# hwaranlee/kaldi-cnn

Measured on AMD Instinct MI355X. Metric: frames/sec fwd+bwd, Conv+Maxpool+FC stack, 4096-frame batch @1/2/4/8 GPU, higher is better.
Workload: dtype f32; 1 GPU; c2: Conv(40x11x3, 8x1, 128) -> Maxpool(1x1x4) -> FC(11616->1024), fwd+bwd+update; frames_per_gpu=4096, parallelism=dp1, global_batch=4096, conv_maxpool_fusion=True, conv_output_stored=False

## Files before the change

### include/kcnn.h

```cpp
#ifndef KCNN_KCNN_H_
#define KCNN_KCNN_H_

#include <stddef.h>
#include <stdint.h>

#include "cnsl-hip-kernels.h"

#ifdef __cplusplus
extern "C" {
#endif

const char *kcnn_last_error(void);
const char *kcnn_version(void);
unsigned long long kcnn_device_malloc_calls(void);
int kcnn_conv_fix_counts(unsigned long long *out, int reset);
int kcnn_init(int device);
int kcnn_set_stream(kcnn_stream_t stream);
int kcnn_synchronize(void);
int kcnn_set_literal_path(int literal);
int kcnn_set_profiling(int on);
int kcnn_set_fusion(int mode);
int kcnn_set_gemm_mode(int mode);
int kcnn_gemm_tile_counts(unsigned long long *out, int reset);
int kcnn_gemm_plan(int trans_a, int trans_b, int m, int n, int k, int lda, int ldb, int *out);
int kcnn_gemm_fixup_counts(unsigned long long *out, int reset);
int kcnn_gemm_fixup_sites_reset(void);
int kcnn_set_kernel_family(const char *name, int value);
int kcnn_get_kernel_family(const char *name);
int kcnn_gemm(int trans_a, int trans_b, int m, int n, int k, float alpha,
              const float *a, int lda, const float *b, int ldb, float beta,
              float *c, int ldc);
int kcnn_split_planes(const float *src, int rows, int cols, int ld, uint16_t *dst, int ldp,
                      int64_t ps);
int kcnn_gemm_planes(int trans_a, int trans_b, int m, int n, int k, float alpha,
                     const uint16_t *a, int lda, int64_t aps, const uint16_t *b, int ldb,
                     int64_t bps, float beta, float *c, int ldc);
int kcnn_profile_string(char *buf, size_t len);
int kcnn_reset_profile(void);
void kcnn_set_randn_seed(uint64_t seed);
int kcnn_selftest_fastdiv(void);

int kcnn_mat_conv2d(const float *in, MatrixDim in_dim, const float *kernel,
                    MatrixDim kernel_dim, int in_height, int in_width,
                    int in_channel, int kernel_height, int kernel_width,
                    int group, float *out, MatrixDim out_dim, int concat);
int kcnn_mat_add_mat_rep_vec(float *m, MatrixDim dim, const float *vec,
                             int vec_dim, int rep);
int kcnn_mat_flip_mat(const float *m, MatrixDim dim, int kernel_height,
                      int kernel_width, int in_channel, int group, float *flip,
                      MatrixDim flip_dim);
int kcnn_mat_padding_zero(const float *m, MatrixDim dim, int orig_height,
                          int orig_width, int orig_channel, int kernel_height,
                          int kernel_width, float *padmat, MatrixDim pad_dim);
int kcnn_mat_tp_block(const float *m, MatrixDim dim, int in_channel,
                      int block_size, float *out, MatrixDim out_dim);
int kcnn_mat_tp_inside_block(const float *m, MatrixDim dim, int group,
                             int block_size, float *out, MatrixDim out_dim);
int kcnn_mat_mod_permute_row(const float *m, MatrixDim dim, int in_channel,
                             int block_size, float *out, MatrixDim out_dim);
int kcnn_mat_mod_permute_channel(float *comp, MatrixDim dim, int comp_idx,
                                 int num_component, int in_height, int in_width,
                                 float *container, MatrixDim container_dim,
                                 int from_comp_to_container);
int kcnn_mat_maxpool_prop(const float *in, MatrixDim in_dim, int in_height,
                          int in_width, int pool_height_dim,
                          int pool_width_dim, int pool_channel_dim,
                          int overlap, int overlap2D, float *out,
                          MatrixDim out_dim);
int kcnn_mat_maxpool_backprop(const float *in_value, MatrixDim in_dim,
                              const float *out_value, MatrixDim ov_dim,
                              const float *out_deriv, MatrixDim od_dim,
                              float *in_deriv, MatrixDim id_dim, int in_height,
                              int in_width, int pool_height_dim,
                              int pool_width_dim, int pool_channel_dim,
                              int overlap, int overlap2D);

typedef struct kcnn_component kcnn_component;

kcnn_component *kcnn_component_new_from_string(const char *initializer_line);
kcnn_component *kcnn_component_read(const char *path);
int kcnn_component_write(const kcnn_component *c, const char *path, int binary);
kcnn_component *kcnn_component_copy(const kcnn_component *c);
void kcnn_component_free(kcnn_component *c);
int kcnn_component_type(const kcnn_component *c, char *buf, size_t len);
int kcnn_component_info(const kcnn_component *c, char *buf, size_t len);
int kcnn_component_input_dim(const kcnn_component *c);
int kcnn_component_output_dim(const kcnn_component *c);
int kcnn_component_context(const kcnn_component *c, int *offsets, int max_len);
int kcnn_component_nonlinear_stats(const kcnn_component *c, double *value_sum,
                                   double *deriv_sum, int max_len, int *len,
                                   double *count);
int kcnn_component_backprop_needs_input(const kcnn_component *c);
int kcnn_component_backprop_needs_output(const kcnn_component *c);
int kcnn_component_propagate(const kcnn_component *c, const float *in,
                             MatrixDim in_dim, float *out, MatrixDim out_dim,
                             int num_chunks);
int kcnn_component_backprop(kcnn_component *c, const float *in_value,
                            MatrixDim in_dim, const float *out_value,
                            MatrixDim ov_dim, const float *out_deriv,
                            MatrixDim od_dim, float *in_deriv,
                            MatrixDim id_dim, int num_chunks, int update);
int kcnn_component_param_dim(const kcnn_component *c, int which, int *rows,
                             int *cols);
int kcnn_component_get_param(const kcnn_component *c, int which, float *dst,
                             MatrixDim dst_dim);
int kcnn_component_set_param(kcnn_component *c, int which, const float *src,
                             MatrixDim src_dim);
float kcnn_component_learning_rate(const kcnn_component *c);
// ... 98 lines not shown
```

### kaldi-cnn_amd/kcnn.py

```python
from __future__ import annotations

import ctypes
import os

_HERE = os.path.dirname(os.path.abspath(__file__))
LIB_PATH = os.environ.get("KCNN_LIB") or os.path.join(_HERE, "libkcnn.so")
INCLUDE_DIR = os.path.join(os.path.dirname(_HERE), "include")


class KcnnError(RuntimeError):
    """A KALDI_ASSERT / KALDI_ERR / HIP error raised inside libkcnn.so."""


class MatrixDim(ctypes.Structure):
    _fields_ = [("rows", ctypes.c_int32), ("cols", ctypes.c_int32),
                ("stride", ctypes.c_int32)]

    def __repr__(self):
        return f"MatrixDim({self.rows}, {self.cols}, {self.stride})"


_lib = None


# ... 84 lines not shown

_initialized_device = None


def init(device: int = 0):
    global _initialized_device
    import torch
    if not torch.cuda.is_available():
        raise KcnnError("no GPU: the kcnn product path has no CPU fallback")
    torch.cuda.set_device(device)
    check(lib().kcnn_init(device))
    sync_stream()
    _initialized_device = device


def sync_stream():
    import torch
    check(lib().kcnn_set_stream(ctypes.c_void_p(torch.cuda.current_stream().cuda_stream)))


def _ensure_init():
    if _initialized_device is None:
        import torch
        init(torch.cuda.current_device() if torch.cuda.is_available() else 0)


def set_literal_path(on: bool):
    check(lib().kcnn_set_literal_path(int(bool(on))))


def set_profiling(on: bool):
    check(lib().kcnn_set_profiling(int(bool(on))))


def set_fusion(mode):
    check(lib().kcnn_set_fusion(int(mode)))


def device_malloc_calls() -> int:
    return int(lib().kcnn_device_malloc_calls())


def conv_fix_counts(reset=False):
    if not hasattr(lib(), "kcnn_conv_fix_counts"):
        return None
    out = (ctypes.c_ulonglong * 3)()
    check(lib().kcnn_conv_fix_counts(out, int(bool(reset))))
    return tuple(int(v) for v in out)


def profile_string() -> str:
    buf = ctypes.create_string_buffer(1 << 16)
    check(lib().kcnn_profile_string(buf, len(buf)))
    return buf.value.decode()


def set_gemm_mode(mode: int):
    check(lib().kcnn_set_gemm_mode(int(mode)))


def gemm_tile_counts(reset=False):
    out = (ctypes.c_ulonglong * 2)()
    check(lib().kcnn_gemm_tile_counts(out, int(bool(reset))))
    return tuple(int(v) for v in out)


def gemm_plan(trans_a, trans_b, m, n, k, lda=None, ldb=None):
    if lda is None:
        lda = m if trans_a else k
    if ldb is None:
        ldb = k if trans_b else n
    out = (ctypes.c_int * 3)()
    check(lib().kcnn_gemm_plan(int(bool(trans_a)), int(bool(trans_b)), int(m), int(n), int(k),
                               int(lda), int(ldb), out))
    return tuple(int(v) for v in out)


def gemm_fixup_counts(reset=False):
    out = (ctypes.c_ulonglong * 2)()
    check(lib().kcnn_gemm_fixup_counts(out, int(bool(reset))))
    return tuple(int(v) for v in out)


def gemm_fixup_sites_reset():
    check(lib().kcnn_gemm_fixup_sites_reset())


def set_kernel_family(name: str, value: int):
    check(lib().kcnn_set_kernel_family(name.encode(), int(value)))


def get_kernel_family(name: str) -> int:
    v = lib().kcnn_get_kernel_family(name.encode())
    if v < 0:
        raise KcnnError(f"unknown kernel family {name!r}")
    return v


def gemm(a, b, c, trans_a=False, trans_b=False, alpha=1.0, beta=0.0):
    m, n = c.shape
    am, k = (a.shape[1], a.shape[0]) if trans_a else (a.shape[0], a.shape[1])
    bk, bn = (b.shape[1], b.shape[0]) if trans_b else (b.shape[0], b.shape[1])
    if am != m or bk != k or bn != n:
        raise KcnnError(f"gemm: op(a) {am}x{k}, op(b) {bk}x{bn} do not make c {m}x{n}")
    for t in (a, b, c):
        dim(t)
    check(lib().kcnn_gemm(int(bool(trans_a)), int(bool(trans_b)), m, n, k,
                          ctypes.c_float(alpha), ctypes.c_void_p(a.data_ptr()), a.stride(0),
                          ctypes.c_void_p(b.data_ptr()), b.stride(0), ctypes.c_float(beta),
                          ctypes.c_void_p(c.data_ptr()), c.stride(0)))


def split_planes(x):
    import torch
    rows, cols = x.shape
    ldp = (cols + 7) // 8 * 8
    out = torch.zeros((3, rows, ldp), dtype=torch.int16, device=x.device)
    check(lib().kcnn_split_planes(ctypes.c_void_p(x.data_ptr()), rows, cols, x.stride(0),
                                  ctypes.c_void_p(out.data_ptr()), ldp,
                                  ctypes.c_int64(rows * ldp)))
    return out


def gemm_planes(ap, bp, c, k, trans_a=False, trans_b=False, alpha=1.0, beta=0.0):
    m, n = c.shape
    check(lib().kcnn_gemm_planes(int(bool(trans_a)), int(bool(trans_b)), m, n, k,
                                 ctypes.c_float(alpha), ctypes.c_void_p(ap.data_ptr()),
                                 ap.stride(1), ctypes.c_int64(ap.stride(0)),
                                 ctypes.c_void_p(bp.data_ptr()), bp.stride(1),
                                 ctypes.c_int64(bp.stride(0)), ctypes.c_float(beta),
                                 ctypes.c_void_p(c.data_ptr()), c.stride(0)))


def reset_profile():
    check(lib().kcnn_reset_profile())


def set_randn_seed(seed: int):
    lib().kcnn_set_randn_seed(ctypes.c_uint64(seed))


def synchronize():
    check(lib().kcnn_synchronize())


def dim(t) -> MatrixDim:
    assert t.dim() == 2, "matrices are 2-D"
    assert t.dtype.is_floating_point and t.element_size() == 4, t.dtype
    assert t.is_cuda, "device tensors only"
    assert t.shape[1] <= 1 or t.stride(1) == 1, "rows must be contiguous"
    stride = t.stride(0) if t.shape[0] > 1 else max(t.shape[1], 1)
    return MatrixDim(t.shape[0], t.shape[1], stride)


def ptr(t):
    return ctypes.c_void_p(t.data_ptr()) if t is not None else None


def empty(rows, cols, device=None):
    import torch
    return torch.empty((rows, cols), dtype=torch.float32,
                       device=device or "cuda")


def zeros(rows, cols, device=None):
    import torch
# ... 668 lines not shown
```

### kaldi-cnn_amd/src/capi/kcnn-capi.cc

```cpp
#include "kcnn.h"

#include <stdlib.h>
#include <string.h>

#include <algorithm>
#include <fstream>
#include <sstream>
#include <string>
#include <utility>
#include <vector>

#include "../cnslmat/hip-util.h"
#include "../kaldi-lite/cu-device.h"
#include "../kaldi-lite/cu-kernels-lite.h"
#include "../kaldi-lite/cu-matrix.h"
#include "../kaldi-lite/kaldi-io.h"
#include "../nnet0/nnet-component-nnet0.h"
#include "../nnet2/nnet-component.h"
#include "../nnet2/nnet-kernels.h"
#include "nnet-stack.h"
#include "online-computer.h"
#include "xent-labels.h"

using namespace kaldi;
// ... 1 lines not shown

struct kcnn_nnet {
  kcnn::NnetStack stack;
  template <typename... Args>
  explicit kcnn_nnet(Args &&...args) : stack(std::forward<Args>(args)...) {}
};

struct kcnn_corpus {
  const float *feats = nullptr;
  MatrixDim dim = {0, 0, 0};
  kcnn::CorpusIndex index;
};

struct kcnn_online {
  kcnn::OnlineComputer computer;
  template <typename... Args>
  explicit kcnn_online(Args &&...args) : computer(std::forward<Args>(args)...) {}
};

namespace {
thread_local std::string g_err;

int fail(const char *what) {
  g_err = what;
  return -1;
}

template <typename F>
int guard(F f) {
  try {
    f();
    return 0;
  } catch (const std::exception &e) {
    return fail(e.what());
  } catch (...) {
    return fail("unknown C++ exception");
  }
}

CuSubMatrix<BaseFloat> view(const float *p, MatrixDim d) {
  return CuSubMatrix<BaseFloat>(const_cast<float *>(p), d.rows, d.cols, d.stride);
}

void borrow(CuMatrix<BaseFloat> *m, const float *p, MatrixDim d) {
  m->Borrow(const_cast<float *>(p), d.rows, d.cols, d.stride);
}

ChunkInfo chunk_info(int cols, int rows, int num_chunks) {
  if (num_chunks <= 0) num_chunks = rows;
  KALDI_ASSERT(rows > 0 && rows % num_chunks == 0);
  return ChunkInfo(cols, num_chunks, 0, rows / num_chunks - 1);
}

void component_chunks(const Component *c, MatrixDim in_dim, MatrixDim out_dim,
                      int num_chunks, ChunkInfo *ii, ChunkInfo *oi) {
  const std::vector<int32> ctx = c->Context();
  if (num_chunks <= 0) num_chunks = out_dim.rows;
  KALDI_ASSERT(out_dim.rows > 0 && out_dim.rows % num_chunks == 0 &&
               in_dim.rows % num_chunks == 0);
  const int ocs = out_dim.rows / num_chunks;
  KALDI_ASSERT(in_dim.rows / num_chunks == ocs + ctx.back() - ctx.front());
  *oi = ChunkInfo(out_dim.cols, num_chunks, 0, ocs - 1);
  if (ctx.front() == 0 && ctx.back() == 0) {
    *ii = ChunkInfo(in_dim.cols, num_chunks, 0, ocs - 1);
  } else {
    *oi = ChunkInfo(out_dim.cols, num_chunks, -ctx.front(), ocs - 1 - ctx.front());
    *ii = ChunkInfo(in_dim.cols, num_chunks, 0, ocs - 1 + ctx.back() - ctx.front());
  }
}

void copy_out(std::string s, char *buf, size_t len) {
  if (!buf || !len) return;
  strncpy(buf, s.c_str(), len - 1);
  buf[len - 1] = '\0';
}

UpdatableComponent *updatable(const kcnn_component *c) {
  KALDI_ASSERT(c && c->c);
  UpdatableComponent *u = dynamic_cast<UpdatableComponent *>(c->c);
  if (!u) KALDI_ERR << c->c->Type() << " has no parameters";
  return u;
}

void param_ref(const kcnn_component *c, int which, float **data, MatrixDim *dim) {
  using cnsl::nnet0::ConvolutionComponent;
  using cnsl::nnet0::FullyConnectedComponent;
  CuMatrixBase<BaseFloat> *m = nullptr;
  CuVectorBase<BaseFloat> *v = nullptr;
  if (auto *cc = dynamic_cast<ConvolutionComponent *>(c->c)) {
    if (which == 0) m = &cc->LinearParamsMutable();
    else if (which == 1) v = &cc->BiasParamsMutable();
    else if (which == 2) m = &cc->PrevGradMutable();
  } else if (auto *fc = dynamic_cast<FullyConnectedComponent *>(c->c)) {
    if (which == 0) m = &fc->LinearParamsMutable();
    else if (which == 1) v = &fc->BiasParamsMutable();
    else if (which == 2) m = &fc->PrevGradMutable();
  } else if (auto *af = dynamic_cast<AffineComponent *>(c->c)) {
    if (which == 0) m = &af->LinearParamsMutable();
    else if (which == 1) v = &af->BiasParamsMutable();
  }
  if (m) {
    *data = m->Data();
    *dim = m->Dim();
  } else if (v) {
    *data = v->Data();
    dim->rows = 1; dim->cols = v->Dim(); dim->stride = v->Dim();
  } else {
    KALDI_ERR << c->c->Type() << " has no parameter #" << which;
  }
}

void copy2d(float *dst, MatrixDim dd, const float *src, MatrixDim sd) {
  KALDI_ASSERT(dd.rows == sd.rows && dd.cols == sd.cols);
  if (dd.rows == 0 || dd.cols == 0) return;
  CU_SAFE_CALL(hipMemcpy2DAsync(dst, sizeof(float) * dd.stride, src,
                                sizeof(float) * sd.stride,
                                sizeof(float) * dd.cols, dd.rows,
                                hipMemcpyDeviceToDevice,
                                CuDevice::Instantiate().Stream()));
}

kcnn::NnetStack &stack(const kcnn_nnet *n) { return const_cast<kcnn_nnet *>(n)->stack; }

void matrix_out(const CuMatrix<BaseFloat> &m, const float **data, MatrixDim *dim) {
  *data = m.Data();
  *dim = m.Dim();
}
}

extern "C" {

const char *kcnn_last_error(void) { return g_err.c_str(); }
const char *kcnn_version(void) { return "kcnn-mi355x 0.1 (gfx950)"; }
unsigned long long kcnn_device_malloc_calls(void) {
  return (unsigned long long)CuDevice::Instantiate().MallocCalls();
}

int kcnn_init(int device) {
  return guard([&] { CuDevice::Instantiate().SelectGpuId("yes", device); });
}
int kcnn_set_stream(kcnn_stream_t stream) {
  return guard([&] {
    CuDevice::Instantiate().SetStream(reinterpret_cast<hipStream_t>(stream));
  });
}
int kcnn_synchronize(void) {
  return guard([&] { CuDevice::Instantiate().Synchronize(); });
}
int kcnn_set_literal_path(int literal) {
  cnsl::nnet0::SetLiteralPath(literal != 0);
  return 0;
}
int kcnn_set_fusion(int on) {
  if (on < 0 || on > 2) return fail("kcnn_set_fusion: mode is 0, 1 or 2");
  kcnn::set_fusion_mode(on);
  return 0;
}
int kcnn_set_gemm_mode(int mode) {
  if (mode < 0 || mode > 4) return fail("kcnn_set_gemm_mode: mode is 0 to 4");
  CuDevice::Instantiate().SetGemmMode(mode);
  return 0;
}
int kcnn_gemm_tile_counts(unsigned long long *out, int reset) {
  if (!out) return fail("kcnn_gemm_tile_counts: out is NULL");
  kl_gemm_f16x3_tile_counts(out, reset);
  return 0;
}
int kcnn_gemm_plan(int trans_a, int trans_b, int m, int n, int k, int lda, int ldb, int *out) {
  if (!out) return fail("kcnn_gemm_plan: out is NULL");
  if (m <= 0 || n <= 0 || k <= 0) return fail("kcnn_gemm_plan: dimensions must be positive");
  kl_gemm_f16x3_plan(trans_a, trans_b, m, n, k, lda, ldb, out);
  return 0;
}
int kcnn_gemm_fixup_counts(unsigned long long *out, int reset) {
  if (!out) return fail("kcnn_gemm_fixup_counts: out is NULL");
  kl_gemm_f16x3_fixup_counts(out, reset);
  return 0;
}
int kcnn_gemm_fixup_sites_reset(void) {
  kl_gemm_f16x3_fixup_sites_reset();
  return 0;
}
int kcnn_set_kernel_family(const char *name, int value) {
  const int f = kcnn::family_by_name(name);
  if (f < 0) return fail("kcnn_set_kernel_family: unknown family");
  if (kcnn::set_family(static_cast<kcnn::Family>(f), value) != 0)
    return fail("kcnn_set_kernel_family: value out of range");
  return 0;
}
int kcnn_get_kernel_family(const char *name) {
  const int f = kcnn::family_by_name(name);
  return f < 0 ? -1 : kcnn::family(static_cast<kcnn::Family>(f));
}
int kcnn_gemm(int trans_a, int trans_b, int m, int n, int k, float alpha,
              const float *a, int lda, const float *b, int ldb, float beta,
              float *c, int ldc) {
  return guard([&] {
    if (m < 0 || n < 0 || k < 0) KALDI_ERR << "kcnn_gemm: negative dimension";
    const int ar = trans_a ? k : m, ac = trans_a ? m : k;
    const int br = trans_b ? n : k, bc = trans_b ? k : n;
    if (lda < ac || ldb < bc || ldc < n) KALDI_ERR << "kcnn_gemm: leading dimension too small";
    CuSubMatrix<BaseFloat> A(const_cast<float *>(a), ar, ac, lda);
    CuSubMatrix<BaseFloat> B(const_cast<float *>(b), br, bc, ldb);
    CuSubMatrix<BaseFloat> C(c, m, n, ldc);
    C.AddMatMat(alpha, A, trans_a ? kTrans : kNoTrans, B, trans_b ? kTrans : kNoTrans, beta);
  });
}
int kcnn_split_planes(const float *src, int rows, int cols, int ld, uint16_t *dst, int ldp,
                      int64_t ps) {
  return guard([&] {
    CuDevice &d = CuDevice::Instantiate();
    const int rc = kl_split_planes(src, rows, cols, ld, dst, ldp, ps,
                                   reinterpret_cast<kcnn_stream_t>(d.Stream()));
    if (rc) KALDI_ERR << "kcnn_split_planes: " << hipGetErrorString((hipError_t)rc);
  });
}
int kcnn_gemm_planes(int trans_a, int trans_b, int m, int n, int k, float alpha,
                     const uint16_t *a, int lda, int64_t aps, const uint16_t *b, int ldb,
                     int64_t bps, float beta, float *c, int ldc) {
  return guard([&] {
    CuDevice &d = CuDevice::Instantiate();
    const size_t wsb = kl_gemm_planes_workspace_bytes(m, n, k);
    CuScratch ws_s(wsb);
    void *ws = ws_s.p;
    const int rc = kl_gemm_planes(trans_a, trans_b, m, n, k, alpha, a, lda, aps, b, ldb, bps,
                                  beta, c, ldc, ws, wsb,
                                  reinterpret_cast<kcnn_stream_t>(d.Stream()));
    if (rc) KALDI_ERR << "kcnn_gemm_planes: " << hipGetErrorString((hipError_t)rc);
  });
}
int kcnn_set_profiling(int on) {
  CuDevice::Instantiate().SetProfiling(on != 0);
  return 0;
}
int kcnn_profile_string(char *buf, size_t len) {
  return guard([&] { copy_out(CuDevice::Instantiate().ProfileString(), buf, len); });
}
int kcnn_reset_profile(void) {
  return guard([&] {
    CuDevice &d = CuDevice::Instantiate();
    (void)d.ProfileString();
    d.ResetProfile();
  });
}
void kcnn_set_randn_seed(uint64_t seed) { SetRandnSeed(seed); }

int kcnn_selftest_fastdiv(void) {
  const uint32_t divs[] = {1, 2, 3, 5, 7, 8, 11, 24, 33, 40, 128, 363, 440,
                           1320, 11616, 46464, 65535, 1000003, 0x7fffffffu};
  uint64_t state = 12345;
  for (uint32_t d : divs) {
    kcnn::FastDiv f(d);
    for (int t = 0; t < 20000; t++) {
      state = state * 6364136223846793005ull + 1442695040888963407ull;
      uint32_t n = (uint32_t)(state >> 33);
      if (t < 64) n = (uint32_t)t;
      if (t >= 64 && t < 128) n = 0x7fffffffu - (uint32_t)(t - 64);
      uint32_t q, r;
      f.divmod(n, q, r);
// ... 160 lines not shown
  guard([&] {
    const std::vector<int32> ctx = c->c->Context();
    n = (int)ctx.size();
    for (int k = 0; k < n && k < max_len; k++) offsets[k] = ctx[k];
  });
  return n;
}
int kcnn_component_nonlinear_stats(const kcnn_component *c, double *value_sum,
                                   double *deriv_sum, int max_len, int *len,
                                   double *count) {
  return guard([&] {
    auto *nl = dynamic_cast<const kaldi::nnet2::NonlinearComponent *>(c->c);
    if (!nl) KALDI_ERR << c->c->Type() << " is not a NonlinearComponent";
    Vector<double> v, d;
    nl->GetValueSum(&v);
    nl->GetDerivSum(&d);
    *len = v.Dim();
    for (int k = 0; k < v.Dim() && k < max_len; k++) {
      value_sum[k] = v(k);
      deriv_sum[k] = d(k);
    }
    *count = nl->Count();
  });
}
int kcnn_component_backprop_needs_input(const kcnn_component *c) {
  return c->c->BackpropNeedsInput();
}
int kcnn_component_backprop_needs_output(const kcnn_component *c) {
  return c->c->BackpropNeedsOutput();
}

int kcnn_component_propagate(const kcnn_component *c, const float *in,
                             MatrixDim in_dim, float *out, MatrixDim out_dim,
                             int num_chunks) {
  return guard([&] {
    auto x = view(in, in_dim), y = view(out, out_dim);
    ChunkInfo ii, oi;
    component_chunks(c->c, in_dim, out_dim, num_chunks, &ii, &oi);
    c->c->Propagate(ii, oi, x, &y);
  });
}

int kcnn_component_backprop(kcnn_component *c, const float *in_value,
                            MatrixDim in_dim, const float *out_value,
                            MatrixDim ov_dim, const float *out_deriv,
                            MatrixDim od_dim, float *in_deriv,
                            MatrixDim id_dim, int num_chunks, int update) {
  return guard([&] {
    auto x = view(in_value, in_dim), y = view(out_value, ov_dim),
         dy = view(out_deriv, od_dim);
    ChunkInfo ii, oi;
    component_chunks(c->c, in_dim, od_dim, num_chunks, &ii, &oi);
    CuMatrix<BaseFloat> dx;
    if (in_deriv) borrow(&dx, in_deriv, id_dim);
    Component *to_update = update ? c->c : nullptr;
    c->c->Backprop(ii, oi, x, y, dy, to_update, in_deriv ? &dx : nullptr);
  });
}

int kcnn_component_param_dim(const kcnn_component *c, int which, int *rows,
                             int *cols) {
  return guard([&] {
    float *p;
    MatrixDim d;
    param_ref(c, which, &p, &d);
    *rows = d.rows;
    *cols = d.cols;
  });
}
int kcnn_component_get_param(const kcnn_component *c, int which, float *dst,
                             MatrixDim dst_dim) {
  return guard([&] {
    float *p;
    MatrixDim d;
    param_ref(c, which, &p, &d);
    copy2d(dst, dst_dim, p, d);
  });
}
int kcnn_component_set_param(kcnn_component *c, int which, const float *src,
                             MatrixDim src_dim) {
  return guard([&] {
    float *p;
    MatrixDim d;
    param_ref(c, which, &p, &d);
    copy2d(p, d, src, src_dim);
  });
}
float kcnn_component_learning_rate(const kcnn_component *c) {
  float lr = -1.0f;
  guard([&] { lr = updatable(c)->LearningRate(); });
  return lr;
}
int kcnn_component_set_learning_rate(kcnn_component *c, float lr) {
  return guard([&] { updatable(c)->SetLearningRate(lr); });
}
int kcnn_component_dot_product(const kcnn_component *a, const kcnn_component *b,
                               float *out) {
  return guard([&] { *out = updatable(a)->DotProduct(*updatable(b)); });
}
int kcnn_component_set_zero(kcnn_component *c, int treat_as_gradient) {
  return guard([&] { updatable(c)->SetZero(treat_as_gradient != 0); });
}
int kcnn_component_scale(kcnn_component *c, float scale) {
  return guard([&] { updatable(c)->Scale(scale); });
}
int kcnn_component_add(kcnn_component *c, float alpha, const kcnn_component *other) {
  return guard([&] { updatable(c)->Add(alpha, *updatable(other)); });
}
int kcnn_component_perturb_params(kcnn_component *c, float stddev) {
  return guard([&] { updatable(c)->PerturbParams(stddev); });
}
int kcnn_component_num_gradient_params(const kcnn_component *c) {
  auto *u = dynamic_cast<UpdatableComponent *>(c->c);
  return u ? u->NumGradientParams() : 0;
}
int kcnn_component_compute_gradient(const kcnn_component *c,
                                    const float *in_value, MatrixDim in_dim,
                                    const float *out_deriv, MatrixDim od_dim,
                                    float *grad) {
  return guard([&] {
    updatable(c)->ComputeGradient(view(in_value, in_dim), view(out_deriv, od_dim),
                                  grad);
  });
}
int kcnn_component_apply_gradient(kcnn_component *c, const float *grad,
                                  int num_sample) {
  return guard([&] { updatable(c)->ApplyGradient(grad, num_sample); });
}
int kcnn_component_backprop_gradient(const kcnn_component *c,
                                     const float *in_value, MatrixDim in_dim,
                                     const float *out_deriv, MatrixDim od_dim,
                                     float *in_deriv, MatrixDim id_dim,
                                     float *grad) {
  return guard([&] {
    const UpdatableComponent *u = updatable(c);
    ChunkInfo ii = chunk_info(in_dim.cols, in_dim.rows, 0);
    ChunkInfo oi = chunk_info(od_dim.cols, od_dim.rows, 0);
    auto x = view(in_value, in_dim);
    CuMatrix<BaseFloat> dx;
    if (in_deriv) borrow(&dx, in_deriv, id_dim);
    u->BackpropGradient(ii, oi, x, x, view(out_deriv, od_dim),
                        in_deriv ? &dx : nullptr, grad);
  });
}
int kcnn_component_conv_flip_branch(const kcnn_component *c) {
  auto *cc = dynamic_cast<cnsl::nnet0::ConvolutionComponent *>(c->c);
  if (!cc) return fail("not a ConvolutionComponent");
  return cc->FlipKernelBranch() ? 1 : 0;
}

namespace {
DropoutComponent *dropout(const kcnn_component *c) {
  KALDI_ASSERT(c && c->c);
  DropoutComponent *d = dynamic_cast<DropoutComponent *>(c->c);
  if (!d) KALDI_ERR << c->c->Type() << " is not a DropoutComponent";
  return d;
}
}

int kcnn_component_set_dropout_scale(kcnn_component *c, float scale) {
  return guard([&] { dropout(c)->SetDropoutScale(scale); });
}
int kcnn_component_dropout_seed(const kcnn_component *c, uint64_t *seed) {
  return guard([&] { *seed = dropout(c)->Seed(); });
}
int kcnn_component_set_dropout_seed(kcnn_component *c, uint64_t seed) {
  return guard([&] { dropout(c)->SetSeed(seed); });
// ... 256 lines not shown
```

### kaldi-cnn_amd/src/capi/nnet-stack.cc

```cpp
#include "nnet-stack.h"

#include <stdlib.h>

#include <cmath>
#include <set>
#include <sstream>
#include <string>

#include "../kaldi-lite/kaldi-io.h"
#include "../nnet2/nnet-kernels.h"
#include "xent-labels.h"

using namespace kaldi;
using namespace kaldi::nnet2;

namespace kcnn {

namespace {
int g_fusion = [] {
  const char *e = getenv("KCNN_FUSE");
  return e && *e ? atoi(e) : 1;
}();

void size_output(CuMatrix<BaseFloat> *m, int rows, int cols) {
// ... 363 lines not shown
}

void NnetStack::MaterialisePoolDeriv(int i) {
  Comp &c = comps_[i];
  KALDI_ASSERT(c.pool != NULL && c.mask_valid && i + 1 < NumComponents());
  c.pool->BackpropFromMask(static_cast<unsigned char *>(c.mask.p), c.pool->OutputDim(),
                           out_deriv_of(i, nullptr, MatrixDim()), &c.deriv);
  c.deriv_deferred = false;
}

const CuMatrix<BaseFloat> &NnetStack::InputDeriv(int i) {
  KALDI_ASSERT(i >= 0 && i < NumComponents());
  if (i == 0 && frames_fused_)
    KALDI_ERR << "input derivative of component 0: after kcnn_nnet_propagate_frames a first "
              << "SpliceComponent reads the corpus itself and its Backprop is not run (it has "
              << "no parameters, and examples share corpus rows)";
  if (comps_[i].deriv_deferred) MaterialisePoolDeriv(i);
  return comps_[i].deriv;
}

void NnetStack::BackpropComponent(int i, const float *out_deriv, MatrixDim od_dim,
                                  BackpropMode mode, float *grad, bool skip_first_dx) {
  const int nc = NumComponents();
  KALDI_ASSERT(i >= 0 && i < nc);
  RequireTrainingForward("kcnn_nnet_backprop_component");
  RequireLastNotFused(i, "kcnn_nnet_backprop_component");
  if (i == 0 && frames_fused_) return;
  Comp &c = comps_[i];
  auto hint = input_stats(i);
  if (out(i).stale == kRecomputable) out(i).stale = kGone;
  const CuMatrix<BaseFloat> &x = in(i).value, &y = out(i).value;
  const bool pool_above_deferred = i + 1 < nc && comps_[i + 1].deriv_deferred;
  CuMatrix<BaseFloat> *dx = &c.deriv;
  if (i == 0 && skip_first_dx && c.updatable) dx = nullptr;
  if (mode == kGradientOnly) {
    KALDI_ASSERT(c.updatable != NULL && grad != NULL && !pool_above_deferred && !c.mask_valid);
    c.updatable->BackpropGradient(in_info(i), out_info(i), x, y,
                                  out_deriv_of(i, out_deriv, od_dim), nullptr, grad);
    return;
  }
  if (pool_above_deferred) {
    const Comp &p = comps_[i + 1];
    if (c.conv && p.pool &&
        c.conv->BackpropPooled(x, *p.pool, static_cast<unsigned char *>(p.mask.p),
                               p.pool->OutputDim(), out_deriv_of(i + 1, out_deriv, od_dim),
                               to_update(c, mode), dx, mode == kGradient ? grad : nullptr))
      return;
    MaterialisePoolDeriv(i + 1);
  }
  CuSubMatrix<BaseFloat> od = out_deriv_of(i, out_deriv, od_dim);
  ChunkInfo ii = in_info(i), oi = out_info(i);
  if (mode == kGradient && c.updatable) {
    c.updatable->BackpropGradient(ii, oi, x, y, od, dx, grad);
    return;
  }
  if (c.mask_valid) {
    KALDI_ASSERT(c.pool != NULL);
    if (g_fusion == 1 && i < nc - 1 && c.pool->FoldsIntoConvBackprop()) {
      c.deriv_deferred = true;
      return;
    }
    c.pool->BackpropFromMask(static_cast<unsigned char *>(c.mask.p), c.pool->OutputDim(), od,
                             dx);
    return;
  }
  c.c->Backprop(ii, oi, x, y, od, to_update(c, mode), dx);
}

void NnetStack::BackpropSplit(int i, const float *out_deriv, MatrixDim od_dim, float *grad,
                              bool skip_first_dx, void (*between)(void *), void *ctx) {
  const int nc = NumComponents();
  KALDI_ASSERT(i >= 0 && i < nc && grad != NULL);
  RequireTrainingForward("kcnn_nnet_backprop_split");
  RequireLastNotFused(i, "kcnn_nnet_backprop_split");
  Comp &c = comps_[i];
  if (c.affine == NULL) KALDI_ERR << "kcnn_nnet_backprop_split: component " << i << " is not affine";
  KALDI_ASSERT(!(i + 1 < nc && comps_[i + 1].deriv_deferred) && !c.mask_valid);
  auto hint = input_stats(i);
  if (out(i).stale == kRecomputable) out(i).stale = kGone;
  const CuMatrix<BaseFloat> &x = in(i).value, &y = out(i).value;
  CuSubMatrix<BaseFloat> od = out_deriv_of(i, out_deriv, od_dim);
  CuMatrix<BaseFloat> *dx = (i == 0 && skip_first_dx) ? nullptr : &c.deriv;
  ChunkInfo ii = in_info(i), oi = out_info(i);
  CuGemmBackpropStats stats(od, c.affine->LinearParams(), true, &x);
  c.affine->BackpropGradient(ii, oi, x, y, od, nullptr, grad);
  if (between) between(ctx);
  if (dx) c.c->Backprop(ii, oi, x, y, od, to_update(c, kDataOnly), dx);
}

void NnetStack::Backprop(const float *out_deriv, MatrixDim od_dim) {
  for (int i = NumComponents() - 1; i >= 0; i--)
    BackpropComponent(i, out_deriv, od_dim, kUpdate, nullptr, false);
}

double *NnetStack::objf_totals() {
  kaldi::CuBuffer &t = labels_.totals;
  if (!t.p)
    CU_SAFE_CALL(hipMemsetAsync(t.reserve(2 * sizeof(double)), 0, 2 * sizeof(double),
                                CuDevice::Instantiate().Stream()));
  return static_cast<double *>(t.p);
}

const char *NnetStack::LabelStaging::Stage(const int32_t *rows, const int32_t *cols,
                                           const float *weights, int num, int num_rows,
                                           hipStream_t st) {
  const size_t bytes = label_layout(num, num_rows).bytes;
  stage_labels(rows, cols, weights, num, num_rows, Begin(bytes));
  return Commit(bytes, st);
}

char *NnetStack::LabelStaging::Begin(size_t bytes) {
  if (copied == nullptr)
    CU_SAFE_CALL(hipEventCreateWithFlags(&copied, hipEventDisableTiming));
  else
    CU_SAFE_CALL(hipEventSynchronize(copied));
  if (host_bytes < bytes) {
    if (host) CU_SAFE_CALL(hipHostFree(host));
    host = nullptr;
    host_bytes = 0;
    CU_SAFE_CALL(hipHostMalloc(&host, bytes, hipHostMallocDefault));
    host_bytes = bytes;
  }
  return static_cast<char *>(host);
}

const char *NnetStack::LabelStaging::Commit(size_t bytes, hipStream_t st) {
  dev.reserve(bytes);
  CU_SAFE_CALL(hipMemcpyAsync(dev.p, host, bytes, hipMemcpyHostToDevice, st));
  CU_SAFE_CALL(hipEventRecord(copied, st));
  return static_cast<const char *>(dev.p);
}

int NnetStack::XentDeriv(const int32_t *rows, const int32_t *cols, const float *weights,
                         int num, const float **out_deriv, MatrixDim *od_dim,
                         const char *who) {
  const int nc = NumComponents();
  RequireTrainingForward(who);
  const Comp &last = comps_[nc - 1];
  const CuMatrix<BaseFloat> &y = out(nc - 1).value;
  const int N = y.NumRows(), dim = last.c->OutputDim();
  if (N == 0 || y.NumCols() != dim) KALDI_ERR << who << ": no Propagate ran";
  if (num > 0 && weights == nullptr) KALDI_ERR << who << ": bad label arrays";
  const std::string bad = check_labels(rows, cols, num, N, dim, true);
  if (!bad.empty()) KALDI_ERR << who << ": " << bad;
  const DeviceLabels lab = StageLabels(rows, cols, weights, num, N);
  const int32_t *d_start = lab.row_start, *d_row = lab.row, *d_col = lab.col;
  const float *d_w = lab.weight;
  double *tot = objf_totals();
  if (last.softmax != nullptr && !cnsl::nnet0::LiteralPath()) {
    last.softmax->BackpropXent(y, d_start, d_col, d_w, tot, last.softmax,
                               &comps_[nc - 1].deriv);
    xent_fused_ = true;
    *out_deriv = nullptr;
    *od_dim = MatrixDim{0, 0, 0};
    return nc - 2;
  }
  xent_deriv_.Resize(N, dim, kSetZero);
  if (num > 0)
    comp_objf_and_deriv(d_row, d_col, d_w, num, y.Data(), y.Dim(), xent_deriv_.Data(),
                        xent_deriv_.Dim(), tot);
  *out_deriv = xent_deriv_.Data();
  *od_dim = xent_deriv_.Dim();
  return nc - 1;
}

void NnetStack::BackpropXent(const int32_t *rows, const int32_t *cols, const float *weights,
// ... 274 lines not shown
```

### kaldi-cnn_amd/src/kaldi-lite/cu-f16-stats.hip

```cpp
#include <hip/hip_runtime.h>
#include <stdint.h>

#include <algorithm>

#include "cnslmat/f16-split.h"
#include "cnslmat/hip-util.h"
#include "cnslmat/pool-stats-dev.h"
#include "cnslmat/pool-stats.h"
#include "kaldi-lite/cu-kernels-lite.h"
#include "kaldi-lite/f16-stats.h"

using namespace kcnn::f16x3;

namespace {

using kcnn::COLMAX_ROWS;
using kcnn::PoolCountSmem;
using kcnn::pool_colmax_block;
using kcnn::pool_count_block;

__device__ __forceinline__ const float *X_row(const StatOp &o, int r) {
  return o.X + (int64_t)r * o.ld;
}

// ... 27 lines not shown
  const int lane = threadIdx.x & 63, wave = threadIdx.x >> 6;
  const bool wide = o.rpb == 1;
  const int r = wide ? blk : blk * 4 + wave;
  if (r >= o.rows) return;
  const float *x = X_row(o, r);
  const int step = wide ? 1024 : 256;
  const int c0 = (wide ? threadIdx.x : lane) * 4;
  const bool held = o.vec && o.cols <= RV * step;
  float4 q[RV];
  uint32_t m = 0, n = 0xffffffffu;
  if (held) {
#pragma unroll
    for (int j = 0; j < RV; ++j) {
      const int c = c0 + j * step;
      if (c + 4 <= o.cols) {
        q[j] = *reinterpret_cast<const float4 *>(x + c);
      } else {
        q[j].x = c < o.cols ? x[c] : 0.0f;
        q[j].y = c + 1 < o.cols ? x[c + 1] : 0.0f;
        q[j].z = c + 2 < o.cols ? x[c + 2] : 0.0f;
        q[j].w = 0.0f;
      }
    }
#pragma unroll
    for (int j = 0; j < RV; ++j) mm4(m, n, q[j]);
  } else {
    int c = c0;
    if (o.vec) {
      for (; c + 3 * step + 4 <= o.cols; c += 4 * step) {
        float4 v[4];
#pragma unroll
        for (int j = 0; j < 4; ++j) v[j] = *reinterpret_cast<const float4 *>(x + c + j * step);
#pragma unroll
        for (int j = 0; j < 4; ++j) mm4(m, n, v[j]);
      }
      for (; c + 4 <= o.cols; c += step) mm4(m, n, *reinterpret_cast<const float4 *>(x + c));
    }
    for (; c < o.cols; c += step)
#pragma unroll
      for (int i = 0; i < 4; ++i)
        if (c + i < o.cols) mm1(m, n, x[c + i]);
  }
#pragma unroll
  for (int d = 32; d >= 1; d >>= 1) {
    m = max(m, (uint32_t)__shfl_xor((int)m, d));
    n = min(n, (uint32_t)__shfl_xor((int)n, d));
  }
  if (wide) {
    if (lane == 0) {
      red[wave] = m;
      red[4 + wave] = n;
    }
    __syncthreads();
    m = max(max(red[0], red[1]), max(red[2], red[3]));
    n = min(min(red[4], red[5]), min(red[6], red[7]));
  }
  uint32_t cnt = 0;
  if (kcnn::f16x3::spread(m, n + 1u)) {
    const float bound = kcnn::f16x3::small_bound(m);
    if (held) {
      auto small = [&](float v) { return (fabsf(v) < bound && v != 0.0f) ? 1u : 0u; };
#pragma unroll
      for (int j = 0; j < RV; ++j)
        cnt += small(q[j].x) + small(q[j].y) + small(q[j].z) + small(q[j].w);
    } else {
      cnt = count_small_row(o, x, bound, c0, step);
    }
#pragma unroll
    for (int d = 32; d >= 1; d >>= 1) cnt += (uint32_t)__shfl_xor((int)cnt, d);
    if (wide) {
      __syncthreads();
      if (lane == 0) red[8 + wave] = cnt;
      __syncthreads();
      cnt = red[8] + red[9] + red[10] + red[11];
    }
  }
  if (wide ? threadIdx.x == 0 : lane == 0) {
    o.out[r] = m;
    o.out[o.rows + r] = n + 1u;
    o.out[2 * (size_t)o.rows + r] = cnt;
  }
}

__device__ __forceinline__ void stats_cols(const StatOp &o, int blk) {
  const int cbi = blk % o.cb, rci = blk / o.cb;
  const int c0 = cbi * 1024 + threadIdx.x * 4;
  const int r0 = rci * o.rb, rend = min(o.rows, r0 + o.rb);
  if (c0 >= o.cols) return;
  const bool v4 = o.vec && c0 + 4 <= o.cols;
  uint32_t cm[4] = {0u, 0u, 0u, 0u};
  uint32_t cn[4] = {0xffffffffu, 0xffffffffu, 0xffffffffu, 0xffffffffu};
  auto load = [&](int r) {
    const float *x = X_row(o, r) + c0;
    if (v4) return *reinterpret_cast<const float4 *>(x);
    float4 q;
    q.x = x[0];
    q.y = c0 + 1 < o.cols ? x[1] : 0.0f;
    q.z = c0 + 2 < o.cols ? x[2] : 0.0f;
    q.w = c0 + 3 < o.cols ? x[3] : 0.0f;
    return q;
  };
  auto take = [&](float4 q) {
    mm1(cm[0], cn[0], q.x);
    mm1(cm[1], cn[1], q.y);
    mm1(cm[2], cn[2], q.z);
    mm1(cm[3], cn[3], q.w);
  };
  int r = r0;
  for (; r + 8 <= rend; r += 8) {
    float4 q[8];
#pragma unroll
    for (int j = 0; j < 8; ++j) q[j] = load(r + j);
#pragma unroll
    for (int j = 0; j < 8; ++j) take(q[j]);
  }
  for (; r < rend; ++r) take(load(r));
  uint32_t *dst = o.part + (size_t)rci * o.cols + c0;
  uint32_t *dsn = dst + (size_t)o.rbk * o.cols;
#pragma unroll
  for (int i = 0; i < 4; ++i)
    if (c0 + i < o.cols) {
      dst[i] = cm[i];
      dsn[i] = cn[i];
    }
}

struct StatOps {
  StatOp o[3];
  PoolColDeferred pc;
  int pcx, pcy, pcn;
};
template <typename Count>
__device__ __forceinline__ int pick_op(const StatOps &s, int blk, Count count, int &local) {
  const int n0 = count(s.o[0]), n1 = count(s.o[1]);
  if (blk < n0) { local = blk; return 0; }
  if (blk < n0 + n1) { local = blk - n0; return 1; }
  local = blk - n0 - n1;
  return 2;
}
__host__ __device__ inline int ncount_blocks(const StatOp &o);
__host__ __device__ inline int nfinal_blocks(const StatOp &o) {
  return o.mode == 1 && o.blocks ? o.fblocks : 0;
}

__global__ __launch_bounds__(256) void stats_kernel(StatOps s) {
  __shared__ uint32_t red[12];
  if (s.o[0].clear && blockIdx.x == 0 && threadIdx.x < 2) s.o[0].clear[threadIdx.x] = 0u;
  const int nb3 = s.o[0].blocks + s.o[1].blocks + s.o[2].blocks;
  if ((int)blockIdx.x >= nb3) {
    const int k = blockIdx.x - nb3;
    pool_colmax_block(s.pc.pcol, s.pc.nblk, s.pc.npool, s.pc.colblk, k % s.pcx, k / s.pcx);
    return;
  }
  int blk;
  const int w = pick_op(s, blockIdx.x, [](const StatOp &o) { return o.blocks; }, blk);
  const StatOp &o = s.o[w];
  if (o.mode == 0) stats_rows(o, blk, red);
  else stats_cols(o, blk);
}

__global__ __launch_bounds__(256) void stats_finalize_kernel(StatOps s) {
  __shared__ uint32_t red[2][4][64];
  __shared__ PoolCountSmem psm;
  const int nf3 = nfinal_blocks(s.o[0]) + nfinal_blocks(s.o[1]) + nfinal_blocks(s.o[2]);
  if ((int)blockIdx.x >= nf3) {
    pool_count_block(s.pc.P, s.pc.ps, s.pc.R, s.pc.npool, s.pc.vec, s.pc.rowblk, s.pc.colblk,
                     blockIdx.x - nf3, s.pcn, psm);
    return;
  }
  int blk;
  const StatOp &o = s.o[pick_op(s, blockIdx.x, [](const StatOp &q) { return nfinal_blocks(q); }, blk)];
  const int lane = threadIdx.x & 63, grp = threadIdx.x >> 6;
  const int c = blk * 64 + lane;
  uint32_t m = 0, n = 0xffffffffu;
  if (c < o.cols) {
    const uint32_t *pm = o.part + c, *pn = o.part + (size_t)o.rbk * o.cols + c;
    int q = grp;
    for (; q + 28 < o.rbk; q += 32) {
      uint32_t a[8], b[8];
#pragma unroll
      for (int j = 0; j < 8; ++j) {
        a[j] = pm[(size_t)(q + 4 * j) * o.cols];
        b[j] = pn[(size_t)(q + 4 * j) * o.cols];
      }
#pragma unroll
      for (int j = 0; j < 8; ++j) {
        m = max(m, a[j]);
        n = min(n, b[j]);
      }
    }
    for (; q < o.rbk; q += 4) {
      m = max(m, pm[(size_t)q * o.cols]);
      n = min(n, pn[(size_t)q * o.cols]);
    }
  }
  red[0][grp][lane] = m;
  red[1][grp][lane] = n;
  __syncthreads();
  m = max(max(red[0][0][lane], red[0][1][lane]), max(red[0][2][lane], red[0][3][lane]));
  n = min(min(red[1][0][lane], red[1][1][lane]), min(red[1][2][lane], red[1][3][lane]));
  if (grp == 0 && c < o.cols) {
    o.out[c] = m;
    o.out[o.cols + c] = n + 1u;
    o.out[2 * (size_t)o.cols + c] = 0;
  }
}

constexpr int CNT_ROWS = 64;
__host__ __device__ inline int ncount_blocks(const StatOp &o) {
  return o.mode == 1 && o.blocks ? ((o.cols + 63) / 64) * ((o.rows + CNT_ROWS - 1) / CNT_ROWS) : 0;
}
__global__ __launch_bounds__(256) void stats_count_kernel(StatOps s) {
  int blk;
  const StatOp &o = s.o[pick_op(s, blockIdx.x, [](const StatOp &q) { return ncount_blocks(q); }, blk)];
  const int ncb = (o.cols + 63) / 64;
  const int cb = blk % ncb, rc = blk / ncb;
  const int lane = threadIdx.x & 63, wave = threadIdx.x >> 6;
  const int c = cb * 64 + lane;
  bool spr = false;
  float bound = 0.0f;
  if (c < o.cols) {
    const uint32_t mx = o.out[c];
    spr = kcnn::f16x3::spread(mx, o.out[o.cols + c]);
    if (spr) bound = kcnn::f16x3::small_bound(mx);
  }
  if (__ballot(spr) == 0) return;
  const int r0 = rc * CNT_ROWS, r1 = min(o.rows, r0 + CNT_ROWS);
  uint32_t cnt = 0;
  if (spr) {
    float v[CNT_ROWS / 4];
#pragma unroll
    for (int i = 0; i < CNT_ROWS / 4; ++i) {
      const int r = r0 + wave + 4 * i;
      v[i] = r < r1 ? fabsf(X_row(o, r)[c]) : 0.0f;
    }
#pragma unroll
    for (int i = 0; i < CNT_ROWS / 4; ++i) cnt += (v[i] < bound && v[i] != 0.0f) ? 1u : 0u;
  }
  if (cnt) atomicAdd(o.out + 2 * (size_t)o.cols + c, cnt);
}

int stats_launch3(const StatOps &ops, hipStream_t st) {
  for (const StatOp &o : ops.o)
    if (o.blocks == 0 && o.out) {
      const size_t n = o.mode == 0 ? (size_t)std::max(o.rows, 0) : (size_t)std::max(o.cols, 0);
      if (n && hipMemsetAsync(o.out, 0, 3 * n * 4, st) != hipSuccess) return (int)hipGetLastError();
    }
  int nb = 0, nf = 0, nc = 0;
  for (const StatOp &o : ops.o) {
    nb += o.blocks;
    nf += nfinal_blocks(o);
    nc += ncount_blocks(o);
  }
  nb += ops.pcx * ops.pcy;
  nf += ops.pcn;
  if (nb == 0) return 0;
  hipLaunchKernelGGL(stats_kernel, dim3(nb), dim3(256), 0, st, ops);
  int rc = kcnn::launch_status();
  if (rc || nf == 0) return rc;
  hipLaunchKernelGGL(stats_finalize_kernel, dim3(nf), dim3(256), 0, st, ops);
  rc = kcnn::launch_status();
  if (rc || nc == 0) return rc;
  hipLaunchKernelGGL(stats_count_kernel, dim3(nc), dim3(256), 0, st, ops);
  return kcnn::launch_status();
}

}

namespace kcnn::f16x3 {

StatOp stat_op(const float *X, int rows, int cols, int ld, int mode, uint32_t *out,
               uint32_t *part) {
  StatOp o{};
  o.X = X; o.out = out; o.part = part;
  o.rows = rows; o.cols = cols; o.ld = ld; o.mode = mode;
  o.vec = ld % 4 == 0 && (uintptr_t)X % 16 == 0;
  if (rows <= 0 || cols <= 0) return o;
  if (mode == 0) {
    o.rpb = cols >= 2048 ? 1 : 4;
    o.blocks = (rows + o.rpb - 1) / o.rpb;
  } else {
    o.cb = (cols + 1023) / 1024;
    o.rbk = std::max(1, std::min(256, std::min((rows + 15) / 16, (1024 + o.cb - 1) / o.cb)));
    o.rb = (rows + o.rbk - 1) / o.rbk;
    o.rbk = (rows + o.rb - 1) / o.rb;
    o.blocks = o.cb * o.rbk;
    o.fblocks = (cols + 63) / 64;
  }
  return o;
}
size_t stat_part_words(int rows, int cols, int mode) {
  if (mode == 0) return 0;
  const StatOp o = stat_op(nullptr, rows, cols, cols, 1, nullptr, nullptr);
  return 2 * (size_t)o.rbk * cols;
}
int stats_launch(const StatOp &a, const StatOp &b, hipStream_t st) {
  StatOps ops{};
  ops.o[0] = a;
  ops.o[1] = b;
  ops.o[2] = StatOp{};
  return stats_launch3(ops, st);
}

}

extern "C" int kl_absmax_rows(const float *X, int rows, int cols, int ld, uint32_t *rmax,
                              kcnn_stream_t stream) {
  if (rows < 0 || cols < 0 || ld < cols || !rmax) return (int)hipErrorInvalidValue;
  return stats_launch(stat_op(X, rows, cols, ld, 0, rmax, nullptr), StatOp{},
                      kcnn::as_stream(stream));
}
extern "C" size_t kl_absmax_cols_words(int rows, int cols) {
  if (rows <= 0 || cols <= 0) return 0;
  return stat_part_words(rows, cols, 1);
}
extern "C" int kl_absmax_cols(const float *X, int rows, int cols, int ld, uint32_t *cmax,
                              uint32_t *part, kcnn_stream_t stream) {
  if (rows < 0 || cols < 0 || ld < cols || !cmax) return (int)hipErrorInvalidValue;
  if (rows > 0 && cols > 0 && !part) return (int)hipErrorInvalidValue;
  return stats_launch(stat_op(X, rows, cols, ld, 1, cmax, part), StatOp{},
                      kcnn::as_stream(stream));
}

extern "C" int kl_absmax_rows_cols(const float *R, int rows, int cols, int ld, uint32_t *rmax,
                                   const float *Q, int qrows, int qcols, int ldq, uint32_t *cmax,
                                   uint32_t *part, uint32_t *clear, kcnn_stream_t stream) {
  if (rows < 0 || cols < 0 || ld < cols || !rmax || qrows < 0 || qcols < 0 || ldq < qcols ||
      !cmax)
    return (int)hipErrorInvalidValue;
  if (qrows > 0 && qcols > 0 && !part) return (int)hipErrorInvalidValue;
  StatOp q = stat_op(Q, qrows, qcols, ldq, 1, cmax, part);
  q.clear = clear;
  const StatOp r = stat_op(R, rows, cols, ld, 0, rmax, nullptr);
  if (clear && q.blocks + r.blocks == 0) {
    const hipError_t e = hipMemsetAsync(clear, 0, 8, kcnn::as_stream(stream));
    if (e != hipSuccess) return (int)e;
  }
  return stats_launch(q, r, kcnn::as_stream(stream));
}

extern "C" int kl_gemm_stats3(const float *X0, int rows0, int cols0, int ld0, int mode0,
                              uint32_t *out0, uint32_t *part0, const float *X1, int rows1,
                              int cols1, int ld1, int mode1, uint32_t *out1, uint32_t *part1,
                              const float *X2, int rows2, int cols2, int ld2, int mode2,
                              uint32_t *out2, uint32_t *part2, void *pool_cols,
                              kcnn_stream_t stream) {
  StatOps ops{};
  if (pool_cols) {
    ops.pc = *static_cast<const PoolColDeferred *>(pool_cols);
    const int ncq = ops.pc.npool % 4 == 0 ? ops.pc.npool / 4 : ops.pc.npool;
    ops.pcx = (ncq + 255) / 256;
    ops.pcy = (ops.pc.nblk + COLMAX_ROWS - 1) / COLMAX_ROWS;
    ops.pcn = std::min(ops.pc.R, 256);
  }
  const float *X[3] = {X0, X1, X2};
  const int rows[3] = {rows0, rows1, rows2}, cols[3] = {cols0, cols1, cols2};
  const int ld[3] = {ld0, ld1, ld2}, mode[3] = {mode0, mode1, mode2};
  uint32_t *out[3] = {out0, out1, out2}, *part[3] = {part0, part1, part2};
  for (int i = 0; i < 3; ++i) {
    ops.o[i] = StatOp{};
    if (!X[i]) continue;
    if (rows[i] < 0 || cols[i] < 0 || ld[i] < cols[i] || !out[i] || (mode[i] != 0 && mode[i] != 1) ||
        (mode[i] == 1 && rows[i] > 0 && cols[i] > 0 && !part[i]))
      return (int)hipErrorInvalidValue;
    ops.o[i] = stat_op(X[i], rows[i], cols[i], ld[i], mode[i], out[i], mode[i] ? part[i] : nullptr);
  }
  return stats_launch3(ops, kcnn::as_stream(stream));
}
```

### kaldi-cnn_amd/src/kaldi-lite/cu-kernels-lite.h

```cpp
#ifndef KCNN_KALDI_LITE_CU_KERNELS_LITE_H_
#define KCNN_KALDI_LITE_CU_KERNELS_LITE_H_

#include <stddef.h>
#include <stdint.h>

#include "cnsl-hip-kernels.h"

#ifdef __cplusplus
extern "C" {
#endif
int kl_set(float *d, MatrixDim dim, float v, kcnn_stream_t st);
int kl_scale(float *d, MatrixDim dim, float a, kcnn_stream_t st);
int kl_add(float *d, MatrixDim dim, float a, kcnn_stream_t st);
int kl_add_mat(float alpha, const float *A, MatrixDim ad, int transA,
               float beta, float *D, MatrixDim dd, kcnn_stream_t st);
int kl_copy_rows_from_vec(const float *v, float *D, MatrixDim dd,
                          kcnn_stream_t st);
int kl_sum_partials(const float *parts, int S, int m, int n, float beta,
                    float *C, MatrixDim cd, kcnn_stream_t st);
size_t kl_col_sum_workspace_bytes(MatrixDim md);
int kl_col_sum(const float *M, MatrixDim md, float alpha, float beta, float *v,
               void *ws, kcnn_stream_t st);
size_t kl_gemm_x6_workspace_bytes(int M, int N, int K);
int kl_gemm_x6(int transA, int transB, int M, int N, int K, float alpha,
               const float *A, int lda, const float *B, int ldb, float beta,
               float *C, int ldc, void *ws, size_t ws_bytes, kcnn_stream_t st);
int kl_absmax_rows(const float *X, int rows, int cols, int ld, uint32_t *rmax,
                   kcnn_stream_t st);
size_t kl_absmax_cols_words(int rows, int cols);
int kl_absmax_cols(const float *X, int rows, int cols, int ld, uint32_t *cmax, uint32_t *part,
                   kcnn_stream_t st);
int kl_absmax_rows_cols(const float *R, int rows, int cols, int ld, uint32_t *rmax,
                        const float *Q, int qrows, int qcols, int ldq, uint32_t *cmax,
                        uint32_t *part, uint32_t *clear, kcnn_stream_t stream);
int kl_gemm_stats3(const float *X0, int rows0, int cols0, int ld0, int mode0, uint32_t *out0,
                   uint32_t *part0, const float *X1, int rows1, int cols1, int ld1, int mode1,
                   uint32_t *out1, uint32_t *part1, const float *X2, int rows2, int cols2,
                   int ld2, int mode2, uint32_t *out2, uint32_t *part2, void *pool_cols,
                   kcnn_stream_t stream);
size_t kl_gemm_f16x3_workspace_bytes(int M, int N, int K);
void kl_gemm_f16x3_tile_counts(unsigned long long *out, int reset);
size_t kl_gemm_f16x3_plan(int transA, int transB, int M, int N, int K, int lda, int ldb,
                          int *out);
void kl_gemm_f16x3_fixup_counts(unsigned long long *out, int reset);
void kl_gemm_f16x3_fixup_sites_reset(void);
size_t kl_gemm_f16x3_full_workspace_bytes(int M, int N, int K);
int kl_gemm_f16x3(int transA, int transB, int M, int N, int K, float alpha,
                  const float *A, int lda, const float *B, int ldb, float beta, float *C,
                  int ldc, void *ws, size_t ws_bytes, kcnn_stream_t st);
int kl_gemm_f16x3_bias(int transA, int transB, int M, int N, int K, float alpha,
                       const float *A, int lda, const float *B, int ldb, float beta, float *C,
                       int ldc, const uint32_t *amax_given, const uint32_t *bmax_given,
                       const float *bias, void *ws, size_t ws_bytes, kcnn_stream_t stream);
int kl_gemm_f16x3_momentum(int transA, int transB, int M, int N, int K, const float *A,
                           int lda, const float *B, int ldb, const uint32_t *amax_given,
                           const uint32_t *bmax_given, float *W, int ldw, float *prev, int ldp,
                           float momentum, float a_wd, float a_g, void *ws, size_t ws_bytes,
                           kcnn_stream_t stream);
int kl_split_planes(const float *src, int rows, int cols, int ld, uint16_t *dst, int ldp,
                    int64_t ps, kcnn_stream_t st);
size_t kl_gemm_planes_workspace_bytes(int M, int N, int K);
int kl_gemm_planes(int transA, int transB, int M, int N, int K, float alpha,
                   const uint16_t *A, int lda, int64_t aps, const uint16_t *B, int ldb,
                   int64_t bps, float beta, float *C, int ldc, void *ws, size_t ws_bytes,
                   kcnn_stream_t st);
int kl_dot(const float *A, MatrixDim ad, const float *B, MatrixDim bd,
           int transB, double *out_dev, kcnn_stream_t st);
#ifdef __cplusplus
}
#endif
#endif
```

### kaldi-cnn_amd/src/kaldi-lite/cu-matrix.cc

```cpp
#include "cu-matrix.h"

#include <math.h>
#include <stdint.h>
#include <stdlib.h>
#include <string.h>

#include <limits>
#include <mutex>
#include <sstream>

#include "cu-device.h"
#include "cu-kernels-lite.h"
#include "../cnslmat/pool-stats.h"
#include "kaldi-io.h"

namespace kaldi {

namespace {
inline kcnn_stream_t S() {
  return reinterpret_cast<kcnn_stream_t>(CuDevice::Instantiate().Stream());
}
inline MatrixIndexT PaddedStride(MatrixIndexT cols) {
  return (cols + 15) / 16 * 16;
}
::MatrixDim VecDim(MatrixIndexT n) {
  ::MatrixDim d;
  d.rows = 1; d.cols = n; d.stride = n;
  return d;
}

std::mutex g_rng_mu;
uint64_t g_rng_state = 20261015ull;
uint64_t splitmix64() {
  uint64_t z = (g_rng_state += 0x9E3779B97F4A7C15ull);
  z = (z ^ (z >> 30)) * 0xBF58476D1CE4E5B9ull;
  z = (z ^ (z >> 27)) * 0x94D049BB133111EBull;
  return z ^ (z >> 31);
}
}

void SetRandnSeed(uint64_t seed) {
  std::lock_guard<std::mutex> lk(g_rng_mu);
  g_rng_state = seed;
}

uint64_t RandU64() {
  std::lock_guard<std::mutex> lk(g_rng_mu);
  return splitmix64();
}

void RandnFill(float *dst, size_t n) {
  std::lock_guard<std::mutex> lk(g_rng_mu);
  for (size_t i = 0; i < n; i += 2) {
    const double u1 = ((splitmix64() >> 11) + 1.0) * (1.0 / 9007199254740993.0);
    const double u2 = (splitmix64() >> 11) * (1.0 / 9007199254740992.0);
    const double r = sqrt(-2.0 * log(u1));
    dst[i] = (float)(r * cos(2.0 * M_PI * u2));
    if (i + 1 < n) dst[i + 1] = (float)(r * sin(2.0 * M_PI * u2));
  }
}

template <typename Real>
void MatrixBase<Real>::Write(std::ostream &os, bool binary) const {
  if (binary) {
    WriteToken(os, binary, sizeof(Real) == 4 ? "FM" : "DM");
    WriteBasicType(os, binary, (int32)rows_);
    WriteBasicType(os, binary, (int32)cols_);
    os.write(reinterpret_cast<const char *>(data_.data()),
             sizeof(Real) * data_.size());
  } else {
    if (cols_ == 0) {
      os << " [ ]\n";
    } else {
      os << " [";
      os.precision(std::numeric_limits<Real>::max_digits10);
      for (MatrixIndexT i = 0; i < rows_; i++) {
        os << "\n  ";
        for (MatrixIndexT j = 0; j < cols_; j++) os << (*this)(i, j) << " ";
      }
      os << "]\n";
    }
  }
  if (os.fail()) KALDI_ERR << "failed to write matrix";
}

template <typename Real>
void MatrixBase<Real>::Read(std::istream &is, bool binary) {
  if (binary) {
    std::string tok;
// ... 114 lines not shown

template <typename Real>
void CuMatrixBase<Real>::CopyFromMat(const CuMatrixBase<Real> &src,
                                     MatrixTransposeType trans) {
  if (trans == kNoTrans) {
    KALDI_ASSERT(src.NumRows() == num_rows_ && src.NumCols() == num_cols_);
    if (num_rows_ == 0 || num_cols_ == 0) return;
    CU_SAFE_CALL(hipMemcpy2DAsync(data_, sizeof(Real) * stride_, src.Data(),
                                  sizeof(Real) * src.Stride(),
                                  sizeof(Real) * num_cols_, num_rows_,
                                  hipMemcpyDeviceToDevice,
                                  CuDevice::Instantiate().Stream()));
  } else {
    KALDI_ASSERT(src.NumCols() == num_rows_ && src.NumRows() == num_cols_);
    CNSL_SAFE_CALL(kl_add_mat(1.0f, src.Data(), src.Dim(), 1, 0.0f, data_, Dim(), S()));
  }
}

template <typename Real>
void CuMatrixBase<Real>::CopyFromMat(const MatrixBase<Real> &src) {
  KALDI_ASSERT(src.NumRows() == num_rows_ && src.NumCols() == num_cols_);
  if (num_rows_ == 0 || num_cols_ == 0) return;
  CU_SAFE_CALL(hipMemcpy2DAsync(data_, sizeof(Real) * stride_, src.Data(),
                                sizeof(Real) * src.Stride(),
                                sizeof(Real) * num_cols_, num_rows_,
                                hipMemcpyHostToDevice,
                                CuDevice::Instantiate().Stream()));
  CuDevice::Instantiate().Synchronize();
}

template <typename Real>
void CuMatrixBase<Real>::CopyToMat(MatrixBase<Real> *dst) const {
  if (dst->NumRows() != num_rows_ || dst->NumCols() != num_cols_)
    dst->Resize(num_rows_, num_cols_);
  if (num_rows_ == 0 || num_cols_ == 0) return;
  CU_SAFE_CALL(hipMemcpy2DAsync(dst->Data(), sizeof(Real) * dst->Stride(),
                                data_, sizeof(Real) * stride_,
                                sizeof(Real) * num_cols_, num_rows_,
                                hipMemcpyDeviceToHost,
                                CuDevice::Instantiate().Stream()));
  CuDevice::Instantiate().Synchronize();
}

template <typename Real>
void CuMatrixBase<Real>::AddMat(Real alpha, const CuMatrixBase<Real> &A,
                                MatrixTransposeType trans) {
  if (trans == kNoTrans)
    KALDI_ASSERT(A.NumRows() == num_rows_ && A.NumCols() == num_cols_);
  else
    KALDI_ASSERT(A.NumCols() == num_rows_ && A.NumRows() == num_cols_);
  CNSL_SAFE_CALL(kl_add_mat(alpha, A.Data(), A.Dim(), trans == kTrans, 1.0f,
                            data_, Dim(), S()));
}

static thread_local const CuGemmStatsHint *g_stats_hints = nullptr;

CuGemmStatsHint::CuGemmStatsHint(const float *data, MatrixIndexT rows, MatrixIndexT cols,
                                 MatrixIndexT stride, const uint32_t *rmax,
                                 const uint32_t *cmax)
    : rowmax(rmax), colmax(cmax), data_(data), rows_(rows), cols_(cols), stride_(stride),
      prev_(g_stats_hints) {
  g_stats_hints = this;
}
CuGemmStatsHint::~CuGemmStatsHint() { g_stats_hints = prev_; }
const CuGemmStatsHint *CuGemmStatsHint::Find(const float *data, MatrixIndexT rows,
                                             MatrixIndexT cols, MatrixIndexT stride) {
  for (const CuGemmStatsHint *h = g_stats_hints; h; h = h->prev_)
    if (h->data_ == data && h->rows_ == rows && h->cols_ == cols && h->stride_ == stride)
      return h;
  return nullptr;
}

static const uint32_t *hint_cols(const CuGemmStatsHint *h, kcnn_stream_t st) {
  if (h->pending) CNSL_SAFE_CALL(kcnn_pool_cols_complete(h->pending, st));
  return h->colmax;
}

CuGemmBackpropStats::CuGemmBackpropStats(const CuMatrixBase<float> &dy,
                                         const CuMatrixBase<float> &W, bool cols,
                                         const CuMatrixBase<float> *in) {
  CuDevice &dev = CuDevice::Instantiate();
  const int N = dy.NumRows(), O = dy.NumCols(), I = W.NumCols();
  if (dev.GemmMode() < 2 || N == 0 || O == 0 || I == 0 || W.NumRows() != O) return;
  {
    const CuGemmStatsHint *hd = CuGemmStatsHint::Find(dy.Data(), N, O, dy.Stride());
    const CuGemmStatsHint *hw = CuGemmStatsHint::Find(W.Data(), O, I, W.Stride());
    if (hd && hd->rowmax && (!cols || hd->colmax) && hw && hw->colmax && !hw->pending) return;
  }
  const size_t pd = cols ? kl_absmax_cols_words(N, O) : 0, pw = kl_absmax_cols_words(O, I);
  const size_t words = 3 * ((size_t)N + O + I) + pd + pw;
  ws_ = dev.Malloc(words * 4);
  uint32_t *rows_d = static_cast<uint32_t *>(ws_), *cols_d = rows_d + 3 * (size_t)N,
           *cols_w = cols_d + 3 * (size_t)O, *part_d = cols_w + 3 * (size_t)I,
           *part_w = part_d + pd;
  PoolColDeferred *pc = nullptr;
  if (cols && in) {
    const CuGemmStatsHint *h =
        CuGemmStatsHint::Find(in->Data(), in->NumRows(), in->NumCols(), in->Stride());
    if (h && h->pending && h->pending->pending) pc = h->pending;
  }
  CNSL_SAFE_CALL(kl_gemm_stats3(dy.Data(), N, O, dy.Stride(), 0, rows_d, nullptr,
                                cols ? dy.Data() : nullptr, N, O, dy.Stride(), 1, cols_d, part_d,
                                W.Data(), O, I, W.Stride(), 1, cols_w, part_w, pc,
                                reinterpret_cast<kcnn_stream_t>(dev.Stream())));
  if (pc) pc->pending = 0;
  hint_d_ = new CuGemmStatsHint(dy.Data(), N, O, dy.Stride(), rows_d, cols ? cols_d : nullptr);
  hint_w_ = new CuGemmStatsHint(W.Data(), O, I, W.Stride(), nullptr, cols_w);
}
CuGemmBackpropStats::~CuGemmBackpropStats() {
  delete hint_w_;
  delete hint_d_;
  if (ws_) CuDevice::Instantiate().Free(ws_);
}

template <typename Real>
bool CuMatrixBase<Real>::GemmF16x3(Real alpha, const CuMatrixBase<Real> &A,
                                   const CuMatrixBase<Real> &Ap, MatrixTransposeType transA,
                                   const CuMatrixBase<Real> &B, const CuMatrixBase<Real> &Bp,
                                   MatrixTransposeType transB, Real beta, const Real *bias) {
  const MatrixIndexT m = num_rows_, n = num_cols_;
  const MatrixIndexT k = transA == kNoTrans ? A.NumCols() : A.NumRows();
  CuDevice &dev0 = CuDevice::Instantiate();
  const CuGemmStatsHint *ha = CuGemmStatsHint::Find(A.Data(), A.NumRows(), A.NumCols(),
                                                    A.Stride());
  const CuGemmStatsHint *hb = CuGemmStatsHint::Find(B.Data(), B.NumRows(), B.NumCols(),
                                                    B.Stride());
  const uint32_t *ag = ha ? (transA == kNoTrans ? ha->rowmax : hint_cols(ha, S())) : nullptr;
  const uint32_t *bg = hb ? (transB == kNoTrans ? hint_cols(hb, S()) : hb->rowmax) : nullptr;
  const size_t wsf = kl_gemm_f16x3_full_workspace_bytes(m, n, k);
  void *wf = dev0.Malloc(wsf);
  const int rc = kl_gemm_f16x3_bias(transA == kTrans, transB == kTrans, m, n, k, alpha,
                                    Ap.Data(), Ap.Stride(), Bp.Data(), Bp.Stride(), beta, data_,
                                    stride_, ag, bg, bias, wf, wsf, S());
  dev0.Free(wf);
  if (rc == (int)hipErrorNotSupported) return false;
  CNSL_SAFE_CALL(rc);
  return true;
}

template <typename Real>
bool CuMatrixBase<Real>::AddMatMatMomentum(const CuMatrixBase<Real> &A,
                                           MatrixTransposeType transA,
                                           const CuMatrixBase<Real> &B,
                                           MatrixTransposeType transB, CuMatrixBase<Real> *prev,
                                           Real momentum, Real a_wd, Real a_g) {
  const MatrixIndexT m = num_rows_, n = num_cols_;
  const MatrixIndexT k = transA == kNoTrans ? A.NumCols() : A.NumRows();
  CuDevice &dev0 = CuDevice::Instantiate();
  auto aligned = [](const CuMatrixBase<Real> &X) {
    return X.Stride() % 4 == 0 && reinterpret_cast<uintptr_t>(X.Data()) % 16 == 0;
  };
  if (dev0.GemmMode() < 2 || m == 0 || n == 0 || k == 0 || !aligned(A) || !aligned(B) ||
      !aligned(*this) || !aligned(*prev))
    return false;
  KALDI_ASSERT((transA == kNoTrans ? A.NumRows() : A.NumCols()) == m &&
               (transB == kNoTrans ? B.NumCols() : B.NumRows()) == n &&
               (transB == kNoTrans ? B.NumRows() : B.NumCols()) == k &&
               prev->NumRows() == m && prev->NumCols() == n);
  CuProfileScope prof("AddMatMat");
  const CuGemmStatsHint *ha = CuGemmStatsHint::Find(A.Data(), A.NumRows(), A.NumCols(),
                                                    A.Stride());
  const CuGemmStatsHint *hb = CuGemmStatsHint::Find(B.Data(), B.NumRows(), B.NumCols(),
                                                    B.Stride());
  const uint32_t *ag = ha ? (transA == kNoTrans ? ha->rowmax : hint_cols(ha, S())) : nullptr;
  const uint32_t *bg = hb ? (transB == kNoTrans ? hint_cols(hb, S()) : hb->rowmax) : nullptr;
  const size_t wsf = kl_gemm_f16x3_full_workspace_bytes(m, n, k);
  void *wf = dev0.Malloc(wsf);
  const int rc = kl_gemm_f16x3_momentum(transA == kTrans, transB == kTrans, m, n, k, A.Data(),
                                        A.Stride(), B.Data(), B.Stride(), ag, bg, data_, stride_,
                                        prev->Data(), prev->Stride(), momentum, a_wd, a_g, wf,
                                        wsf, S());
  dev0.Free(wf);
  if (rc == (int)hipErrorNotSupported) return false;
  CNSL_SAFE_CALL(rc);
  return true;
}

template <typename Real>
void CuMatrixBase<Real>::AddMatMatBias(Real alpha, const CuMatrixBase<Real> &A,
                                       MatrixTransposeType transA, const CuMatrixBase<Real> &B,
                                       MatrixTransposeType transB,
                                       const CuVectorBase<Real> &bias) {
  const MatrixIndexT k = transA == kNoTrans ? A.NumCols() : A.NumRows();
  KALDI_ASSERT(bias.Dim() == num_cols_);
  CuDevice &dev0 = CuDevice::Instantiate();
  auto aligned = [](const CuMatrixBase<Real> &X) {
    return X.Stride() % 4 == 0 && reinterpret_cast<uintptr_t>(X.Data()) % 16 == 0;
  };
  if (dev0.GemmMode() >= 2 && num_rows_ > 0 && num_cols_ > 0 && k > 0 && aligned(A) &&
      aligned(B)) {
// ... 393 lines not shown
```

### kaldi-cnn_amd/src/kaldi-lite/cu-matrix.h

```cpp
#ifndef KCNN_KALDI_LITE_CU_MATRIX_H_
#define KCNN_KALDI_LITE_CU_MATRIX_H_

#include <istream>
#include <ostream>
#include <vector>

#include "cnsl-hip-kernels.h"
#include "kaldi-common.h"

namespace kaldi {

template <typename Real> class CuMatrix;
template <typename Real> class CuSubMatrix;
template <typename Real> class CuVectorBase;
template <typename Real> class CuSubVector;

template <typename Real>
class VectorBase {
 public:
  MatrixIndexT Dim() const { return (MatrixIndexT)data_.size(); }
  Real *Data() { return data_.data(); }
  const Real *Data() const { return data_.data(); }
  Real &operator()(MatrixIndexT i) { return data_[i]; }
  Real operator()(MatrixIndexT i) const { return data_[i]; }
  void Resize(MatrixIndexT d) { data_.assign(d, Real(0)); }
  void Read(std::istream &is, bool binary);
  void Write(std::ostream &os, bool binary) const;

 protected:
  std::vector<Real> data_;
};
template <typename Real>
class Vector : public VectorBase<Real> {
 public:
  Vector() {}
  explicit Vector(MatrixIndexT d) { this->Resize(d); }
};

template <typename Real>
class MatrixBase {
 public:
  MatrixIndexT NumRows() const { return rows_; }
  MatrixIndexT NumCols() const { return cols_; }
  MatrixIndexT Stride() const { return cols_; }
  Real *Data() { return data_.data(); }
  const Real *Data() const { return data_.data(); }
  Real &operator()(MatrixIndexT r, MatrixIndexT c) { return data_[(size_t)r * cols_ + c]; }
  Real operator()(MatrixIndexT r, MatrixIndexT c) const { return data_[(size_t)r * cols_ + c]; }
  void Resize(MatrixIndexT r, MatrixIndexT c) {
    rows_ = r; cols_ = c; data_.assign((size_t)r * c, Real(0));
  }
  void Read(std::istream &is, bool binary);
  void Write(std::ostream &os, bool binary) const;

 protected:
  MatrixIndexT rows_ = 0, cols_ = 0;
  std::vector<Real> data_;
};
template <typename Real>
class Matrix : public MatrixBase<Real> {
 public:
  Matrix() {}
  Matrix(MatrixIndexT r, MatrixIndexT c) { this->Resize(r, c); }
};

template <typename Real>
class CuMatrixBase {
 public:
  MatrixIndexT NumRows() const { return num_rows_; }
  MatrixIndexT NumCols() const { return num_cols_; }
  MatrixIndexT Stride() const { return stride_; }
  ::MatrixDim Dim() const {
    ::MatrixDim d;
    d.rows = num_rows_; d.cols = num_cols_; d.stride = stride_;
    return d;
  }
  Real *Data() { return data_; }
  const Real *Data() const { return data_; }
  Real *RowData(MatrixIndexT r) { return data_ + (int64)r * stride_; }
  const Real *RowData(MatrixIndexT r) const { return data_ + (int64)r * stride_; }

  void SetZero();
  void Set(Real value);
  void Add(Real value);
  void Scale(Real value);
  void SetRandn();
// ... 116 lines not shown
template <typename Real>
class CuVectorBase {
 public:
  MatrixIndexT Dim() const { return dim_; }
  Real *Data() { return data_; }
  const Real *Data() const { return data_; }
  void SetZero();
  void Set(Real v);
  void Add(Real v);
  void Scale(Real v);
  void SetRandn();
  void CopyFromVec(const CuVectorBase<Real> &v);
  void CopyFromVec(const VectorBase<Real> &v);
  void CopyToVec(VectorBase<Real> *v) const;
  void AddVec(Real alpha, const CuVectorBase<Real> &v, Real beta = 1.0);
  void AddRowSumMat(Real alpha, const CuMatrixBase<Real> &M, Real beta = 1.0);
  void CopyColFromMat(const CuMatrixBase<Real> &M, MatrixIndexT col);
  CuSubVector<Real> Range(MatrixIndexT o, MatrixIndexT l) const;
  void Write(std::ostream &os, bool binary) const;

 protected:
  CuVectorBase() : data_(nullptr), dim_(0) {}
  CuVectorBase(Real *d, MatrixIndexT n) : data_(d), dim_(n) {}
  Real *data_;
  MatrixIndexT dim_;

 private:
  KALDI_DISALLOW_COPY_AND_ASSIGN(CuVectorBase);
};

template <typename Real>
class CuVector : public CuVectorBase<Real> {
 public:
  CuVector() {}
  explicit CuVector(MatrixIndexT d, MatrixResizeType t = kSetZero) { Resize(d, t); }
  CuVector(const CuVector<Real> &o) { *this = o; }
  ~CuVector() { Destroy(); }
  CuVector<Real> &operator=(const CuVectorBase<Real> &o);
  CuVector<Real> &operator=(const CuVector<Real> &o);
  CuVector<Real> &operator=(const VectorBase<Real> &o);
  void Resize(MatrixIndexT d, MatrixResizeType t = kSetZero);
  void Read(std::istream &is, bool binary);
  void Borrow(Real *data, MatrixIndexT dim);

 private:
  void Destroy();
  bool borrowed_ = false;
};

template <typename Real>
class CuSubVector : public CuVectorBase<Real> {
 public:
  CuSubVector(Real *d, MatrixIndexT n) : CuVectorBase<Real>(d, n) {}
  CuSubVector(const CuSubVector<Real> &o) : CuVectorBase<Real>(o.data_, o.dim_) {}
};

template <typename Real>
Real TraceMatMat(const CuMatrixBase<Real> &A, const CuMatrixBase<Real> &B,
                 MatrixTransposeType trans = kNoTrans);
template <typename Real>
Real VecVec(const CuVectorBase<Real> &a, const CuVectorBase<Real> &b);

}
struct PoolColDeferred;
namespace kaldi {
class CuGemmStatsHint {
 public:
  CuGemmStatsHint(const float *data, MatrixIndexT rows, MatrixIndexT cols, MatrixIndexT stride,
                  const uint32_t *rowmax, const uint32_t *colmax);
  ~CuGemmStatsHint();
  CuGemmStatsHint(const CuGemmStatsHint &) = delete;
  CuGemmStatsHint &operator=(const CuGemmStatsHint &) = delete;
  static const CuGemmStatsHint *Find(const float *data, MatrixIndexT rows, MatrixIndexT cols,
                                     MatrixIndexT stride);
  const uint32_t *rowmax, *colmax;
  PoolColDeferred *pending = nullptr;

 private:
  const float *data_;
  MatrixIndexT rows_, cols_, stride_;
  const CuGemmStatsHint *prev_;
};

class CuGemmBackpropStats {
 public:
  CuGemmBackpropStats(const CuMatrixBase<float> &out_deriv, const CuMatrixBase<float> &linear,
                      bool cols, const CuMatrixBase<float> *in_value = NULL);
  ~CuGemmBackpropStats();
  CuGemmBackpropStats(const CuGemmBackpropStats &) = delete;
  CuGemmBackpropStats &operator=(const CuGemmBackpropStats &) = delete;

 private:
  void *ws_ = nullptr;
  CuGemmStatsHint *hint_d_ = nullptr, *hint_w_ = nullptr;
};

void RandnFill(float *dst, size_t n);
void SetRandnSeed(uint64_t seed);
uint64_t RandU64();

}

#endif
```

### kaldi-cnn_amd/src/kaldi-lite/f16-stats.h

```cpp
#ifndef KCNN_KALDI_LITE_F16_STATS_H_
#define KCNN_KALDI_LITE_F16_STATS_H_

#include <hip/hip_runtime_api.h>
#include <stddef.h>
#include <stdint.h>

namespace kcnn::f16x3 {

struct StatOp {
  const float *X;
  uint32_t *out;
  uint32_t *part;
  int rows, cols, ld, mode, vec;
  int blocks;
  int rpb;
  int cb, rbk, rb;
  int fblocks;
  uint32_t *clear;
};

StatOp stat_op(const float *X, int rows, int cols, int ld, int mode, uint32_t *out,
               uint32_t *part);
size_t stat_part_words(int rows, int cols, int mode);
int stats_launch(const StatOp &a, const StatOp &b, hipStream_t st);

}

#endif
```

### kaldi-cnn_amd/src/nnet0/nnet-component-nnet0.cc

```cpp
#include "nnet-component-nnet0.h"

#include <math.h>
#include <stdlib.h>

#include <sstream>

#include "../kaldi-lite/cu-device.h"
#include "../kaldi-lite/kaldi-io.h"
#include "../nnet2/parse-from-string.h"
#include "cnsl-hip-kernels.h"
#include "cnslmat/conv-update.h"

namespace cnsl {
namespace nnet0 {

namespace {
bool g_literal = getenv("KCNN_LITERAL") != nullptr && atoi(getenv("KCNN_LITERAL")) != 0;
inline kcnn_stream_t S() {
  return reinterpret_cast<kcnn_stream_t>(CuDevice::Instantiate().Stream());
}
::MatrixDim Dense(int32 rows, int32 cols) {
  ::MatrixDim d;
  d.rows = rows; d.cols = cols; d.stride = cols;
  return d;
// ... 909 lines not shown
  std::ostringstream ostr_beg, ostr_end;
  ostr_beg << "<" << Type() << ">";
  ostr_end << "</" << Type() << ">";
  ExpectOneOrTwoTokens(is, binary, ostr_beg.str(), "<InputDim>");
  ReadBasicType(is, binary, &input_dim_);
  ExpectToken(is, binary, "<in_height>");
  ReadBasicType(is, binary, &in_height_);
  ExpectToken(is, binary, "<in_width>");
  ReadBasicType(is, binary, &in_width_);
  ExpectToken(is, binary, "<in_channel>");
  ReadBasicType(is, binary, &in_channel_);
  ExpectToken(is, binary, "<OutputDim>");
  ReadBasicType(is, binary, &output_dim_);
  ExpectToken(is, binary, "<PoolHeightDim>");
  ReadBasicType(is, binary, &pool_height_dim_);
  ExpectToken(is, binary, "<PoolWidthDim>");
  ReadBasicType(is, binary, &pool_width_dim_);
  ExpectToken(is, binary, "<PoolChannelDim>");
  ReadBasicType(is, binary, &pool_channel_dim_);
  std::string tok;
  ReadToken(is, binary, &tok);
  if (tok == "<Overlap>") {
    ReadBasicType(is, binary, &overlap_);
    ReadToken(is, binary, &tok);
    if (tok == "<Overlap2D>") {
      ReadBasicType(is, binary, &overlap2D_);
      ExpectToken(is, binary, "</MaxpoolComponent>");
    } else {
      overlap2D_ = false;
      KALDI_ASSERT(tok == ostr_end.str());
    }
  } else {
    overlap_ = false;
    overlap2D_ = false;
    KALDI_ASSERT(tok == ostr_end.str());
  }
}

void MaxpoolComponent::Write(std::ostream &os, bool binary) const {
  WriteToken(os, binary, "<MaxpoolComponent>");
  WriteToken(os, binary, "<InputDim>");
  WriteBasicType(os, binary, input_dim_);
  WriteToken(os, binary, "<in_height>");
  WriteBasicType(os, binary, in_height_);
  WriteToken(os, binary, "<in_width>");
  WriteBasicType(os, binary, in_width_);
  WriteToken(os, binary, "<in_channel>");
  WriteBasicType(os, binary, in_channel_);
  WriteToken(os, binary, "<OutputDim>");
  WriteBasicType(os, binary, output_dim_);
  WriteToken(os, binary, "<PoolHeightDim>");
  WriteBasicType(os, binary, pool_height_dim_);
  WriteToken(os, binary, "<PoolWidthDim>");
  WriteBasicType(os, binary, pool_width_dim_);
  WriteToken(os, binary, "<PoolChannelDim>");
  WriteBasicType(os, binary, pool_channel_dim_);
  WriteToken(os, binary, "<Overlap>");
  WriteBasicType(os, binary, overlap_);
  WriteToken(os, binary, "<Overlap2D>");
  WriteBasicType(os, binary, overlap2D_);
  WriteToken(os, binary, "</MaxpoolComponent>");
}

std::string MaxpoolComponent::Info() const {
  std::stringstream stream;
  stream << Type() << " input-dim=" << input_dim_ << " ( in-height="
         << in_height_ << ", in-width=" << in_width_
         << ", in-channels=" << in_channel_ << "), output-dim=" << output_dim_
         << ", pool_height_dim_= " << pool_height_dim_
         << ", pool_width_dim_ = " << pool_width_dim_
         << ", pool_channel_dim_ = " << pool_channel_dim_
         << ", max-pool-overlap_ = " << overlap_
         << ", max-pool-overlap_2D = " << overlap2D_;
  return stream.str();
}

void FullyConnectedComponent::Read(std::istream &is, bool binary) {
  std::ostringstream ostr_beg, ostr_end;
  ostr_beg << "<" << Type() << ">";
  ostr_end << "</" << Type() << ">";
  ExpectOneOrTwoTokens(is, binary, ostr_beg.str(), "<LearningRate>");
  ReadBasicType(is, binary, &learning_rate_);
  ExpectToken(is, binary, "<LinearParams>");
  linear_params_.Read(is, binary);
  ExpectToken(is, binary, "<BiasParams>");
  bias_params_.Read(is, binary);
  ExpectToken(is, binary, "<WeightDecay>");
  ReadBasicType(is, binary, &weight_decay_);
  ExpectToken(is, binary, "<Momentum>");
  ReadBasicType(is, binary, &momentum_);
  ExpectToken(is, binary, "<PrevGrad>");
  prev_grad_.Read(is, binary);
  ExpectToken(is, binary, ostr_end.str());
}

void FullyConnectedComponent::Write(std::ostream &os, bool binary) const {
  std::ostringstream ostr_beg, ostr_end;
  ostr_beg << "<" << Type() << ">";
  ostr_end << "</" << Type() << ">";
  WriteToken(os, binary, ostr_beg.str());
  WriteToken(os, binary, "<LearningRate>");
  WriteBasicType(os, binary, learning_rate_);
  WriteToken(os, binary, "<LinearParams>");
  linear_params_.Write(os, binary);
  WriteToken(os, binary, "<BiasParams>");
  bias_params_.Write(os, binary);
  WriteToken(os, binary, "<WeightDecay>");
  WriteBasicType(os, binary, weight_decay_);
  WriteToken(os, binary, "<Momentum>");
  WriteBasicType(os, binary, momentum_);
  WriteToken(os, binary, "<PrevGrad>");
  prev_grad_.Write(os, binary);
  WriteToken(os, binary, ostr_end.str());
}

void FullyConnectedComponent::Init(BaseFloat learning_rate, int32 input_dim,
                                   int32 output_dim, BaseFloat param_stddev,
                                   BaseFloat bias_stddev,
                                   BaseFloat weight_decay, BaseFloat momentum) {
  UpdatableComponent::Init(learning_rate);
  KALDI_ASSERT(input_dim > 0 && output_dim > 0);
  linear_params_.Resize(output_dim, input_dim);
  bias_params_.Resize(output_dim);
  KALDI_ASSERT(output_dim > 0 && input_dim > 0 && param_stddev >= 0.0);
  linear_params_.SetRandn();
  linear_params_.Scale(param_stddev);
  bias_params_.SetZero();
  bias_params_.Add(bias_stddev);
  weight_decay_ = weight_decay;
  KALDI_ASSERT(weight_decay_ > 0.0);
  momentum_ = momentum;
  KALDI_ASSERT(momentum_ > 0.0);
  prev_grad_.Resize(output_dim, input_dim);
  prev_grad_.SetZero();
}

void FullyConnectedComponent::InitFromString(std::string args) {
  std::string orig_args(args);
  std::string matrix_filename;
  BaseFloat learning_rate = learning_rate_;
  BaseFloat weight_decay = weight_decay_, momentum = momentum_;
  int32 input_dim = -1, output_dim = -1;
  ParseFromString("learning-rate", &args, &learning_rate);
  ParseFromString("weight-decay", &args, &weight_decay);
  ParseFromString("momentum", &args, &momentum);
  if (ParseFromString("matrix", &args, &matrix_filename))
    KALDI_ERR << "matrix= initialisation is not supported (SURVEY B12)";
  bool ok = true;
  ok = ok && ParseFromString("input-dim", &args, &input_dim);
  ok = ok && ParseFromString("output-dim", &args, &output_dim);
  BaseFloat param_stddev = 1.0 / std::sqrt((double)(input_dim > 0 ? input_dim : 1)),
            bias_stddev = 1.0;
  ParseFromString("param-stddev", &args, &param_stddev);
  ParseFromString("bias-stddev", &args, &bias_stddev);
  if (!ok) KALDI_ERR << "Bad initializer " << orig_args;
  Init(learning_rate, input_dim, output_dim, param_stddev, bias_stddev,
       weight_decay, momentum);
  if (!args.empty())
    KALDI_ERR << "Could not process these elements in initializer: " << args;
}

std::string FullyConnectedComponent::Info() const {
  std::stringstream stream;
  const double size = (double)linear_params_.NumRows() * linear_params_.NumCols();
  const double ls = std::sqrt(TraceMatMat(linear_params_, linear_params_, kTrans) / size);
  const double bs = std::sqrt(VecVec(bias_params_, bias_params_) / bias_params_.Dim());
  stream << Type() << ", input-dim=" << InputDim()
         << ", output-dim=" << OutputDim() << ", linear-params-stddev=" << ls
         << ", bias-params-stddev=" << bs
         << ", learning-rate=" << LearningRate()
         << ", weight-decay=" << weight_decay_ << ", momentum=" << momentum_;
  return stream.str();
}

Component *FullyConnectedComponent::Copy() const {
  FullyConnectedComponent *ans = new FullyConnectedComponent();
  ans->learning_rate_ = learning_rate_;
  ans->linear_params_ = linear_params_;
  ans->bias_params_ = bias_params_;
  ans->weight_decay_ = weight_decay_;
  ans->momentum_ = momentum_;
  ans->prev_grad_ = prev_grad_;
  ans->is_gradient_ = is_gradient_;
  return ans;
}

void FullyConnectedComponent::ComputeGradient(const CuMatrixBase<BaseFloat> &in_value,
                                              const CuMatrixBase<BaseFloat> &out_deriv,
                                              BaseFloat *grad) const {
  KALDI_ASSERT(in_value.NumCols() == InputDim() &&
               out_deriv.NumCols() == OutputDim() &&
               in_value.NumRows() == out_deriv.NumRows());
  CuProfileScope prof("FullyConnectedComponent::ComputeGradient");
  CuSubMatrix<BaseFloat> gW(grad, OutputDim(), InputDim(), InputDim());
  gW.AddMatMat(1.0, out_deriv, kTrans, in_value, kNoTrans, 0.0);
  CuSubVector<BaseFloat> gb(grad + (size_t)OutputDim() * InputDim(), OutputDim());
  gb.AddRowSumMat(1.0, out_deriv, 0.0);
}

void FullyConnectedComponent::ApplyGradient(const BaseFloat *grad, int32 num_sample) {
  KALDI_ASSERT(num_sample > 0);
  CuProfileScope prof("FullyConnectedComponent::ApplyGradient");
  const double learning_rate = learning_rate_ / (double)num_sample;
  const BaseFloat a_wd = (BaseFloat)(-1 * learning_rate * weight_decay_);
  const BaseFloat a_g = (BaseFloat)learning_rate;
  CNSL_SAFE_CALL(hipF_momentum_update(
      linear_params_.Data(), linear_params_.Dim(), prev_grad_.Data(),
      prev_grad_.Dim(), grad, Dense(OutputDim(), InputDim()), momentum_, a_wd,
      a_g, bias_params_.Data(), grad + (size_t)OutputDim() * InputDim(),
      OutputDim(), S()));
}

void FullyConnectedComponent::UpdateSimple(const CuMatrixBase<BaseFloat> &in_value,
                                           const CuMatrixBase<BaseFloat> &out_deriv) {
  const int32 num_sample = in_value.NumRows();
  if (LiteralPath()) {
    const double learning_rate = learning_rate_ / (double)num_sample;
    bias_params_.AddRowSumMat(learning_rate, out_deriv, 1.0);
    prev_grad_.Scale(momentum_);
    prev_grad_.AddMat(-1 * learning_rate * weight_decay_, linear_params_, kNoTrans);
    prev_grad_.AddMatMat(learning_rate, out_deriv, kTrans, in_value, kNoTrans, 1.0);
    linear_params_.AddMat(1.0, prev_grad_, kNoTrans);
    return;
  }
  {
    const double learning_rate = learning_rate_ / (double)num_sample;
    const BaseFloat a_wd = (BaseFloat)(-1 * learning_rate * weight_decay_);
    const BaseFloat a_g = (BaseFloat)learning_rate;
    CuProfileScope prof("FullyConnectedComponent::ComputeGradient");
    if (linear_params_.AddMatMatMomentum(out_deriv, kTrans, in_value, kNoTrans, &prev_grad_,
                                         momentum_, a_wd, a_g)) {
      bias_params_.AddRowSumMat(a_g, out_deriv, 1.0);
      return;
    }
  }
  Scratch grad(sizeof(BaseFloat) * (size_t)NumGradientParams());
  ComputeGradient(in_value, out_deriv, grad.f());
  ApplyGradient(grad.f(), num_sample);
}

}
}
```

### kaldi-cnn_amd/src/nnet2/nnet-component.cc

```cpp
#include "nnet-component.h"

#include <math.h>

#include <sstream>

#include "../kaldi-lite/cu-device.h"
#include "../kaldi-lite/kaldi-io.h"
#include "../nnet0/nnet-component-nnet0.h"
#include "nnet-kernels.h"
#include "parse-from-string.h"

namespace kaldi {
namespace nnet2 {

int32 ChunkInfo::GetIndex(int32 offset) const {
  if (offsets_.empty()) return offset - first_offset_;
  for (size_t i = 0; i < offsets_.size(); i++)
    if (offsets_[i] == offset) return (int32)i;
  KALDI_ERR << "could not find offset " << offset;
  return -1;
}
int32 ChunkInfo::GetOffset(int32 index) const {
  if (offsets_.empty()) return first_offset_ + index;
  KALDI_ASSERT(index >= 0 && index < (int32)offsets_.size());
// ... 85 lines not shown
  std::stringstream stream;
  stream << Type() << ", input-dim=" << InputDim()
         << ", output-dim=" << OutputDim() << ", learning-rate=" << LearningRate();
  return stream.str();
}

void ExpectOneOrTwoTokens(std::istream &is, bool binary,
                          const std::string &token1,
                          const std::string &token2) {
  KALDI_ASSERT(token1 != token2);
  std::string temp;
  ReadToken(is, binary, &temp);
  if (temp == token1) {
    ExpectToken(is, binary, token2);
  } else if (temp != token2) {
    KALDI_ERR << "Expecting token " << token1 << " or " << token2
              << " but got " << temp;
  }
}

namespace {
template <typename F>
bool ParseGeneric(const std::string &name, std::string *string, F convert) {
  std::vector<std::string> split_string;
  SplitStringToVector(*string, " \t", true, &split_string);
  const std::string name_equals = name + "=";
  const size_t len = name_equals.length();
  for (size_t i = 0; i < split_string.size(); i++) {
    if (split_string[i].compare(0, len, name_equals) == 0) {
      if (!convert(split_string[i].substr(len)))
        KALDI_ERR << "Bad option " << split_string[i];
      *string = "";
      for (size_t j = 0; j < split_string.size(); j++) {
        if (j != i) {
          if (!string->empty()) *string += " ";
          *string += split_string[j];
        }
      }
      return true;
    }
  }
  return false;
}
}

bool ParseFromString(const std::string &name, std::string *string,
                     int32 *param) {
  return ParseGeneric(name, string, [&](const std::string &v) {
    return ConvertStringToInteger(v, param);
  });
}
bool ParseFromString(const std::string &name, std::string *string,
                     bool *param) {
  return ParseGeneric(name, string, [&](const std::string &b) {
    if (b.empty()) return false;
    if (b[0] == 'f' || b[0] == 'F') *param = false;
    else if (b[0] == 't' || b[0] == 'T') *param = true;
    else return false;
    return true;
  });
}
bool ParseFromString(const std::string &name, std::string *string,
                     BaseFloat *param) {
  return ParseGeneric(name, string, [&](const std::string &v) {
    return ConvertStringToReal(v, param);
  });
}
bool ParseFromString(const std::string &name, std::string *string,
                     std::string *param) {
  return ParseGeneric(name, string, [&](const std::string &v) {
    *param = v;
    return true;
  });
}
bool ParseFromString(const std::string &name, std::string *string,
                     std::vector<int32> *param) {
  return ParseGeneric(name, string, [&](const std::string &v) {
    return SplitStringToIntegers(v, ":", false, param);
  });
}

AffineComponent::AffineComponent(const AffineComponent &component)
    : UpdatableComponent(component),
      linear_params_(component.linear_params_),
      bias_params_(component.bias_params_),
      is_gradient_(component.is_gradient_) {}

AffineComponent::AffineComponent(const CuMatrixBase<BaseFloat> &linear_params,
                                 const CuVectorBase<BaseFloat> &bias_params,
                                 BaseFloat learning_rate)
    : UpdatableComponent(learning_rate),
      linear_params_(linear_params),
      bias_params_(),
      is_gradient_(false) {
  bias_params_ = bias_params;
  KALDI_ASSERT(linear_params.NumRows() == bias_params.Dim() &&
               bias_params.Dim() != 0);
}

void AffineComponent::Init(BaseFloat learning_rate, int32 input_dim,
                           int32 output_dim, BaseFloat param_stddev,
                           BaseFloat bias_stddev) {
  UpdatableComponent::Init(learning_rate);
  linear_params_.Resize(output_dim, input_dim);
  bias_params_.Resize(output_dim);
  KALDI_ASSERT(output_dim > 0 && input_dim > 0 && param_stddev >= 0.0);
  linear_params_.SetRandn();
  linear_params_.Scale(param_stddev);
  bias_params_.SetRandn();
  bias_params_.Scale(bias_stddev);
}

void AffineComponent::InitFromString(std::string args) {
  std::string orig_args(args);
  bool ok = true;
  BaseFloat learning_rate = learning_rate_;
  int32 input_dim = -1, output_dim = -1;
  ParseFromString("learning-rate", &args, &learning_rate);
  ok = ok && ParseFromString("input-dim", &args, &input_dim);
  ok = ok && ParseFromString("output-dim", &args, &output_dim);
  BaseFloat param_stddev = 1.0 / std::sqrt((double)(input_dim > 0 ? input_dim : 1)),
            bias_stddev = 1.0;
  ParseFromString("param-stddev", &args, &param_stddev);
  ParseFromString("bias-stddev", &args, &bias_stddev);
  if (!args.empty())
    KALDI_ERR << "Could not process these elements in initializer: " << args;
  if (!ok) KALDI_ERR << "Bad initializer " << orig_args;
  Init(learning_rate, input_dim, output_dim, param_stddev, bias_stddev);
}

std::string AffineComponent::Info() const {
  std::stringstream stream;
  const double size = (double)linear_params_.NumRows() * linear_params_.NumCols();
  const double ls = std::sqrt(TraceMatMat(linear_params_, linear_params_, kTrans) / size);
  const double bs = std::sqrt(VecVec(bias_params_, bias_params_) / bias_params_.Dim());
  stream << Type() << ", input-dim=" << InputDim()
         << ", output-dim=" << OutputDim() << ", linear-params-stddev=" << ls
         << ", bias-params-stddev=" << bs
         << ", learning-rate=" << LearningRate();
  return stream.str();
}

void AffineComponent::Propagate(const ChunkInfo &in_info,
                                const ChunkInfo &out_info,
                                const CuMatrixBase<BaseFloat> &in,
                                CuMatrixBase<BaseFloat> *out) const {
  in_info.CheckSize(in);
  out_info.CheckSize(*out);
  KALDI_ASSERT(in_info.NumChunks() == out_info.NumChunks());
  out->AddMatMatBias(1.0, in, kNoTrans, linear_params_, kTrans, bias_params_);
}

void AffineComponent::Scale(BaseFloat scale) {
  linear_params_.Scale(scale);
  bias_params_.Scale(scale);
}

void AffineComponent::Add(BaseFloat alpha, const UpdatableComponent &other_in) {
  const AffineComponent *other = dynamic_cast<const AffineComponent *>(&other_in);
  KALDI_ASSERT(other != NULL);
  linear_params_.AddMat(alpha, other->linear_params_);
  bias_params_.AddVec(alpha, other->bias_params_);
}

void AffineComponent::UpdateSimple(const CuMatrixBase<BaseFloat> &in_value,
                                   const CuMatrixBase<BaseFloat> &out_deriv) {
  bias_params_.AddRowSumMat(learning_rate_, out_deriv, 1.0);
  linear_params_.AddMatMat(learning_rate_, out_deriv, kTrans, in_value,
                           kNoTrans, 1.0);
}

void AffineComponent::Backprop(const ChunkInfo &, const ChunkInfo &,
                               const CuMatrixBase<BaseFloat> &in_value,
                               const CuMatrixBase<BaseFloat> &,
                               const CuMatrixBase<BaseFloat> &out_deriv,
                               Component *to_update_in,
                               CuMatrix<BaseFloat> *in_deriv) const {
  AffineComponent *to_update = dynamic_cast<AffineComponent *>(to_update_in);
  in_deriv->Resize(out_deriv.NumRows(), InputDim(), kUndefined);
  CuGemmBackpropStats stats(out_deriv, linear_params_, to_update != NULL, &in_value);
  in_deriv->AddMatMat(1.0, out_deriv, kNoTrans, linear_params_, kNoTrans, 0.0);
  if (to_update != NULL) {
    if (to_update->is_gradient_)
      to_update->UpdateSimple(in_value, out_deriv);
    else
      to_update->Update(in_value, out_deriv);
  }
}

void AffineComponent::SetZero(bool treat_as_gradient) {
  if (treat_as_gradient) {
    SetLearningRate(1.0);
    is_gradient_ = true;
  }
  linear_params_.SetZero();
  bias_params_.SetZero();
}

void AffineComponent::Read(std::istream &is, bool binary) {
  std::ostringstream ostr_beg, ostr_end;
  ostr_beg << "<" << Type() << ">";
  ostr_end << "</" << Type() << ">";
  ExpectOneOrTwoTokens(is, binary, ostr_beg.str(), "<LearningRate>");
  ReadBasicType(is, binary, &learning_rate_);
  ExpectToken(is, binary, "<LinearParams>");
  linear_params_.Read(is, binary);
  ExpectToken(is, binary, "<BiasParams>");
  bias_params_.Read(is, binary);
  std::string tok;
  ReadToken(is, binary, &tok);
  if (tok == "<AvgInput>") {
    CuVector<BaseFloat> avg_input;
    avg_input.Read(is, binary);
    BaseFloat avg_input_count;
    ExpectToken(is, binary, "<AvgInputCount>");
    ReadBasicType(is, binary, &avg_input_count);
    ReadToken(is, binary, &tok);
  }
  if (tok == "<IsGradient>") {
    ReadBasicType(is, binary, &is_gradient_);
    ExpectToken(is, binary, ostr_end.str());
  } else {
    is_gradient_ = false;
    KALDI_ASSERT(tok == ostr_end.str());
  }
}

void AffineComponent::Write(std::ostream &os, bool binary) const {
  std::ostringstream ostr_beg, ostr_end;
  ostr_beg << "<" << Type() << ">";
  ostr_end << "</" << Type() << ">";
  WriteToken(os, binary, ostr_beg.str());
  WriteToken(os, binary, "<LearningRate>");
  WriteBasicType(os, binary, learning_rate_);
  WriteToken(os, binary, "<LinearParams>");
  linear_params_.Write(os, binary);
  WriteToken(os, binary, "<BiasParams>");
  bias_params_.Write(os, binary);
  WriteToken(os, binary, "<IsGradient>");
  WriteBasicType(os, binary, is_gradient_);
  WriteToken(os, binary, ostr_end.str());
}

BaseFloat AffineComponent::DotProduct(const UpdatableComponent &other_in) const {
  const AffineComponent *other = dynamic_cast<const AffineComponent *>(&other_in);
  KALDI_ASSERT(other != NULL);
  return TraceMatMat(linear_params_, other->linear_params_, kTrans) +
         VecVec(bias_params_, other->bias_params_);
}

Component *AffineComponent::Copy() const {
  AffineComponent *ans = new AffineComponent();
  ans->learning_rate_ = learning_rate_;
  ans->linear_params_ = linear_params_;
  ans->bias_params_ = bias_params_;
  ans->is_gradient_ = is_gradient_;
  return ans;
}

void AffineComponent::PerturbParams(BaseFloat stddev) {
  CuMatrix<BaseFloat> temp_linear_params(linear_params_);
  temp_linear_params.SetRandn();
  linear_params_.AddMat(stddev, temp_linear_params);
  CuVector<BaseFloat> temp_bias_params(bias_params_);
  temp_bias_params.SetRandn();
  bias_params_.AddVec(stddev, temp_bias_params);
}

void AffineComponent::SetParams(const VectorBase<BaseFloat> &bias,
                                const MatrixBase<BaseFloat> &linear) {
  bias_params_ = bias;
  linear_params_ = linear;
  KALDI_ASSERT(bias_params_.Dim() == linear_params_.NumRows());
}

int32 AffineComponent::GetParameterDim() const {
  return (InputDim() + 1) * OutputDim();
}
void AffineComponent::Vectorize(VectorBase<BaseFloat> *params) const {
  KALDI_ASSERT(params->Dim() == GetParameterDim());
  Matrix<BaseFloat> W;
  linear_params_.CopyToMat(&W);
  Vector<BaseFloat> b;
  bias_params_.CopyToVec(&b);
  const size_t nw = (size_t)InputDim() * OutputDim();
  std::copy(W.Data(), W.Data() + nw, params->Data());
  std::copy(b.Data(), b.Data() + OutputDim(), params->Data() + nw);
}
void AffineComponent::UnVectorize(const VectorBase<BaseFloat> &params) {
  KALDI_ASSERT(params.Dim() == GetParameterDim());
  Matrix<BaseFloat> W(OutputDim(), InputDim());
  const size_t nw = (size_t)InputDim() * OutputDim();
  std::copy(params.Data(), params.Data() + nw, W.Data());
  Vector<BaseFloat> b(OutputDim());
  std::copy(params.Data() + nw, params.Data() + nw + OutputDim(), b.Data());
  linear_params_.CopyFromMat(W);
  bias_params_.CopyFromVec(b);
}


namespace {
kcnn_stream_t NS() {
  return reinterpret_cast<kcnn_stream_t>(CuDevice::Instantiate().Stream());
}
double *NewDeviceDoubles(int32 n) {
  void *p = CuDevice::Instantiate().Malloc(sizeof(double) * (size_t)n);
  CU_SAFE_CALL(hipMemsetAsync(p, 0, sizeof(double) * (size_t)n,
                              CuDevice::Instantiate().Stream()));
  return static_cast<double *>(p);
}
void FreeDeviceDoubles(double **p) {
  if (*p) CuDevice::Instantiate().Free(*p);
  *p = nullptr;
}
void ReadDeviceDoubles(std::istream &is, bool binary, int32 *dim, double **p) {
  Vector<double> v;
  v.Read(is, binary);
  FreeDeviceDoubles(p);
  *dim = v.Dim();
  if (v.Dim() == 0) return;
  *p = NewDeviceDoubles(v.Dim());
  CU_SAFE_CALL(hipMemcpyAsync(*p, v.Data(), sizeof(double) * v.Dim(), hipMemcpyHostToDevice,
                              CuDevice::Instantiate().Stream()));
  CU_SAFE_CALL(hipStreamSynchronize(CuDevice::Instantiate().Stream()));
}
void DownloadDoubles(const double *p, int32 dim, Vector<double> *v) {
  v->Resize(dim);
  if (dim == 0) return;
  CU_SAFE_CALL(hipMemcpyAsync(v->Data(), p, sizeof(double) * dim, hipMemcpyDeviceToHost,
                              CuDevice::Instantiate().Stream()));
  CU_SAFE_CALL(hipStreamSynchronize(CuDevice::Instantiate().Stream()));
}
}

NonlinearComponent::NonlinearComponent(const NonlinearComponent &other)
    : Component(), dim_(other.dim_), stats_dim_(0), value_sum_(nullptr),
      deriv_sum_(nullptr), count_(other.count_) {
  if (other.stats_dim_ > 0) {
    stats_dim_ = other.stats_dim_;
    value_sum_ = NewDeviceDoubles(stats_dim_);
    deriv_sum_ = NewDeviceDoubles(stats_dim_);
    hipStream_t st = CuDevice::Instantiate().Stream();
    CU_SAFE_CALL(hipMemcpyAsync(value_sum_, other.value_sum_, sizeof(double) * stats_dim_,
                                hipMemcpyDeviceToDevice, st));
    CU_SAFE_CALL(hipMemcpyAsync(deriv_sum_, other.deriv_sum_, sizeof(double) * stats_dim_,
                                hipMemcpyDeviceToDevice, st));
  }
}

NonlinearComponent::~NonlinearComponent() {
  FreeDeviceDoubles(&value_sum_);
  FreeDeviceDoubles(&deriv_sum_);
}

void NonlinearComponent::SetDim(int32 dim) {
  KALDI_ASSERT(dim > 0);
  dim_ = dim;
  FreeDeviceDoubles(&value_sum_);
  FreeDeviceDoubles(&deriv_sum_);
  stats_dim_ = 0;
  EnsureStats();
  count_ = 0.0;
}

void NonlinearComponent::EnsureStats() {
  if (stats_dim_ == dim_ && value_sum_ && deriv_sum_) return;
  FreeDeviceDoubles(&value_sum_);
  FreeDeviceDoubles(&deriv_sum_);
  value_sum_ = NewDeviceDoubles(dim_);
  deriv_sum_ = NewDeviceDoubles(dim_);
  stats_dim_ = dim_;
  count_ = 0.0;
}

void NonlinearComponent::Scale(BaseFloat scale) {
  if (stats_dim_ > 0) {
    CNSL_SAFE_CALL(kn_dvec_update(value_sum_, nullptr, 0.0, scale, stats_dim_, NS()));
    CNSL_SAFE_CALL(kn_dvec_update(deriv_sum_, nullptr, 0.0, scale, stats_dim_, NS()));
  }
// ... 510 lines not shown
```

### kaldi-cnn_amd/src/nnet2/nnet-component.h

```cpp
#ifndef KCNN_NNET2_NNET_COMPONENT_H_
#define KCNN_NNET2_NNET_COMPONENT_H_

#include <atomic>
#include <iostream>
#include <string>
#include <vector>

#include "../kaldi-lite/cu-matrix.h"
#include "../kaldi-lite/kaldi-common.h"

namespace kaldi {
namespace nnet2 {

class ChunkInfo {
 public:
  ChunkInfo() : feat_dim_(0), num_chunks_(0), first_offset_(0), last_offset_(0) {}
  ChunkInfo(int32 feat_dim, int32 num_chunks, int32 first_offset,
            int32 last_offset)
      : feat_dim_(feat_dim), num_chunks_(num_chunks),
        first_offset_(first_offset), last_offset_(last_offset) { Check(); }
  ChunkInfo(int32 feat_dim, int32 num_chunks, const std::vector<int32> offsets)
      : feat_dim_(feat_dim), num_chunks_(num_chunks),
        first_offset_(offsets.front()), last_offset_(offsets.back()),
        offsets_(offsets) {
// ... 41 lines not shown
        out->NumCols() != out_info.NumCols())
      out->Resize(out_info.NumRows(), out_info.NumCols());
    Propagate(in_info, out_info, in, static_cast<CuMatrixBase<BaseFloat> *>(out));
  }
  virtual void Backprop(const ChunkInfo &in_info, const ChunkInfo &out_info,
                        const CuMatrixBase<BaseFloat> &in_value,
                        const CuMatrixBase<BaseFloat> &out_value,
                        const CuMatrixBase<BaseFloat> &out_deriv,
                        Component *to_update,
                        CuMatrix<BaseFloat> *in_deriv) const = 0;
  virtual bool BackpropNeedsInput() const { return true; }
  virtual bool BackpropNeedsOutput() const { return true; }

  static Component *ReadNew(std::istream &is, bool binary);
  virtual Component *Copy() const = 0;
  static Component *NewFromString(const std::string &initializer_line);
  static Component *NewComponentOfType(const std::string &type);
  virtual void Read(std::istream &is, bool binary) = 0;
  virtual void Write(std::ostream &os, bool binary) const = 0;
  virtual std::string Info() const;

 private:
  int32 index_;
  KALDI_DISALLOW_COPY_AND_ASSIGN(Component);
};

class UpdatableComponent : public Component {
 public:
  UpdatableComponent(const UpdatableComponent &other)
      : Component(), learning_rate_(other.learning_rate_) {}
  void Init(BaseFloat learning_rate) { learning_rate_ = learning_rate; }
  UpdatableComponent(BaseFloat learning_rate) { Init(learning_rate); }
  UpdatableComponent() : learning_rate_(0.001) {}
  virtual ~UpdatableComponent() {}
  virtual void SetZero(bool treat_as_gradient) = 0;
  virtual BaseFloat DotProduct(const UpdatableComponent &other) const = 0;
  virtual void PerturbParams(BaseFloat stddev) = 0;
  virtual void Scale(BaseFloat scale) = 0;
  virtual void Add(BaseFloat alpha, const UpdatableComponent &other) = 0;
  void SetLearningRate(BaseFloat lrate) { learning_rate_ = lrate; }
  BaseFloat LearningRate() const { return learning_rate_; }
  virtual std::string Info() const;
  virtual int32 GetParameterDim() const { KALDI_ASSERT(0); return 0; }
  virtual void Vectorize(VectorBase<BaseFloat> *params) const { (void)params; KALDI_ASSERT(0); }
  virtual void UnVectorize(const VectorBase<BaseFloat> &params) { (void)params; KALDI_ASSERT(0); }

  virtual int32 NumGradientParams() const { return 0; }
  virtual void ComputeGradient(const CuMatrixBase<BaseFloat> &in_value,
                               const CuMatrixBase<BaseFloat> &out_deriv,
                               BaseFloat *grad) const {
    (void)in_value; (void)out_deriv; (void)grad;
    KALDI_ERR << Type() << " does not support ComputeGradient";
  }
  virtual void ApplyGradient(const BaseFloat *grad, int32 num_sample) {
    (void)grad; (void)num_sample;
    KALDI_ERR << Type() << " does not support ApplyGradient";
  }
  virtual void BackpropGradient(const ChunkInfo &in_info, const ChunkInfo &out_info,
                                const CuMatrixBase<BaseFloat> &in_value,
                                const CuMatrixBase<BaseFloat> &out_value,
                                const CuMatrixBase<BaseFloat> &out_deriv,
                                CuMatrix<BaseFloat> *in_deriv, BaseFloat *grad) const {
    if (in_deriv != NULL)
      Backprop(in_info, out_info, in_value, out_value, out_deriv, NULL, in_deriv);
    ComputeGradient(in_value, out_deriv, grad);
  }

 protected:
  BaseFloat learning_rate_;

 private:
  const UpdatableComponent &operator=(const UpdatableComponent &other);
};

class AffineComponent : public UpdatableComponent {
  friend class AffineComponentPreconditioned;

 public:
  explicit AffineComponent(const AffineComponent &other);
  AffineComponent(const CuMatrixBase<BaseFloat> &linear_params,
                  const CuVectorBase<BaseFloat> &bias_params,
                  BaseFloat learning_rate);
  AffineComponent() : is_gradient_(false) {}
  virtual int32 InputDim() const { return linear_params_.NumCols(); }
  virtual int32 OutputDim() const { return linear_params_.NumRows(); }
  void Init(BaseFloat learning_rate, int32 input_dim, int32 output_dim,
            BaseFloat param_stddev, BaseFloat bias_stddev);
  virtual void InitFromString(std::string args);
  virtual std::string Info() const;
  virtual std::string Type() const { return "AffineComponent"; }
  virtual bool BackpropNeedsInput() const { return true; }
  virtual bool BackpropNeedsOutput() const { return false; }
  using Component::Propagate;
  virtual void Propagate(const ChunkInfo &in_info, const ChunkInfo &out_info,
                         const CuMatrixBase<BaseFloat> &in,
                         CuMatrixBase<BaseFloat> *out) const;
  virtual void Scale(BaseFloat scale);
  virtual void Add(BaseFloat alpha, const UpdatableComponent &other);
  virtual void Backprop(const ChunkInfo &in_info, const ChunkInfo &out_info,
                        const CuMatrixBase<BaseFloat> &in_value,
                        const CuMatrixBase<BaseFloat> &out_value,
                        const CuMatrixBase<BaseFloat> &out_deriv,
                        Component *to_update,
                        CuMatrix<BaseFloat> *in_deriv) const;
  virtual void SetZero(bool treat_as_gradient);
  virtual void Read(std::istream &is, bool binary);
  virtual void Write(std::ostream &os, bool binary) const;
  virtual BaseFloat DotProduct(const UpdatableComponent &other) const;
  virtual Component *Copy() const;
  virtual void PerturbParams(BaseFloat stddev);
  virtual void SetParams(const VectorBase<BaseFloat> &bias,
                         const MatrixBase<BaseFloat> &linear);
  const CuVector<BaseFloat> &BiasParams() { return bias_params_; }
  const CuMatrix<BaseFloat> &LinearParams() { return linear_params_; }
  virtual int32 GetParameterDim() const;
  virtual void Vectorize(VectorBase<BaseFloat> *params) const;
  virtual void UnVectorize(const VectorBase<BaseFloat> &params);

  CuMatrix<BaseFloat> &LinearParamsMutable() { return linear_params_; }
  CuVector<BaseFloat> &BiasParamsMutable() { return bias_params_; }

 protected:
  virtual void Update(const CuMatrixBase<BaseFloat> &in_value,
                      const CuMatrixBase<BaseFloat> &out_deriv) {
    UpdateSimple(in_value, out_deriv);
  }
  virtual void UpdateSimple(const CuMatrixBase<BaseFloat> &in_value,
                            const CuMatrixBase<BaseFloat> &out_deriv);
  const AffineComponent &operator=(const AffineComponent &other);

  CuMatrix<BaseFloat> linear_params_;
  CuVector<BaseFloat> bias_params_;
  bool is_gradient_;
};


class NonlinearComponent : public Component {
 public:
  void Init(int32 dim) { dim_ = dim; count_ = 0.0; }
  explicit NonlinearComponent(int32 dim) : value_sum_(nullptr), deriv_sum_(nullptr) {
    Init(dim);
  }
  NonlinearComponent() : dim_(0), stats_dim_(0), value_sum_(nullptr),
                         deriv_sum_(nullptr), count_(0.0) {}
  explicit NonlinearComponent(const NonlinearComponent &other);
  virtual ~NonlinearComponent();
  virtual int32 InputDim() const { return dim_; }
  virtual int32 OutputDim() const { return dim_; }
  virtual void InitFromString(std::string args);
  virtual void Read(std::istream &is, bool binary);
  virtual void Write(std::ostream &os, bool binary) const;
  void Scale(BaseFloat scale);
  void Add(BaseFloat alpha, const NonlinearComponent &other);
  void GetValueSum(Vector<double> *v) const;
  void GetDerivSum(Vector<double> *v) const;
  double Count() const { return count_; }
  void SetDim(int32 dim);

 protected:
  friend class RectifiedLinearComponent;
  friend class SoftmaxComponent;
  void EnsureStats();
  int32 dim_;
  int32 stats_dim_;
  double *value_sum_;
  double *deriv_sum_;
  double count_;

 private:
  const NonlinearComponent &operator=(const NonlinearComponent &other);
};

class RectifiedLinearComponent : public NonlinearComponent {
 public:
  explicit RectifiedLinearComponent(int32 dim) : NonlinearComponent(dim) {}
  explicit RectifiedLinearComponent(const RectifiedLinearComponent &other)
      : NonlinearComponent(other) {}
  RectifiedLinearComponent() {}
  virtual std::string Type() const { return "RectifiedLinearComponent"; }
  virtual Component *Copy() const { return new RectifiedLinearComponent(*this); }
  virtual bool BackpropNeedsInput() const { return false; }
  virtual bool BackpropNeedsOutput() const { return true; }
  using Component::Propagate;
  virtual void Propagate(const ChunkInfo &in_info, const ChunkInfo &out_info,
                         const CuMatrixBase<BaseFloat> &in,
                         CuMatrixBase<BaseFloat> *out) const;
  virtual void Backprop(const ChunkInfo &in_info, const ChunkInfo &out_info,
                        const CuMatrixBase<BaseFloat> &in_value,
                        const CuMatrixBase<BaseFloat> &out_value,
                        const CuMatrixBase<BaseFloat> &out_deriv,
                        Component *to_update,
                        CuMatrix<BaseFloat> *in_deriv) const;

 private:
  RectifiedLinearComponent &operator=(const RectifiedLinearComponent &other);
};

class SpliceComponent : public Component {
 public:
  SpliceComponent() : input_dim_(0), const_component_dim_(0) {}
  void Init(int32 input_dim, std::vector<int32> context, int32 const_component_dim = 0);
  virtual std::string Type() const { return "SpliceComponent"; }
  virtual std::string Info() const;
  virtual void InitFromString(std::string args);
  virtual int32 InputDim() const { return input_dim_; }
  virtual int32 OutputDim() const;
  virtual std::vector<int32> Context() const { return context_; }
  using Component::Propagate;
  virtual void Propagate(const ChunkInfo &in_info, const ChunkInfo &out_info,
                         const CuMatrixBase<BaseFloat> &in,
                         CuMatrixBase<BaseFloat> *out) const;
  virtual void Backprop(const ChunkInfo &in_info, const ChunkInfo &out_info,
                        const CuMatrixBase<BaseFloat> &in_value,
                        const CuMatrixBase<BaseFloat> &out_value,
                        const CuMatrixBase<BaseFloat> &out_deriv,
                        Component *to_update,
// ... 133 lines not shown
```

Before: 3.106 million frames/sec.

## Cache FC weight absmax stats and fuse row/col stats with in-kernel small-value counting

Adds a per-component weight statistics cache, invalidated whenever the weights are obtained for mutation, and hands it as a hint to the split-precision GEMMs in forward and backward so they do not recompute weight column/row absmax stats on every call. A new fused stats path computes row and column partial maxima in one pass. It also folds the separate small-value count kernel into the finalize kernel, which rescans only suspect row blocks, removing one launch. The risk is stale stats if any weight write bypasses MutableW, for example through direct pointer access from the C API.

```diff
diff --git a/include/kcnn.h b/include/kcnn.h
--- a/include/kcnn.h
+++ b/include/kcnn.h
@@ -24,6 +24,7 @@
 int kcnn_gemm_tile_counts(unsigned long long *out, int reset);
 int kcnn_gemm_plan(int trans_a, int trans_b, int m, int n, int k, int lda, int ldb, int *out);
 int kcnn_gemm_fixup_counts(unsigned long long *out, int reset);
+int kcnn_fc_wstats_counts(unsigned long long *out, int reset);
 int kcnn_gemm_fixup_sites_reset(void);
 int kcnn_set_kernel_family(const char *name, int value);
 int kcnn_get_kernel_family(const char *name);
diff --git a/kaldi-cnn_amd/kcnn.py b/kaldi-cnn_amd/kcnn.py
--- a/kaldi-cnn_amd/kcnn.py
+++ b/kaldi-cnn_amd/kcnn.py
@@ -190,6 +190,12 @@
     return tuple(int(v) for v in out)
 
 
+def fc_wstats_counts(reset=False):
+    out = (ctypes.c_ulonglong * 2)()
+    check(lib().kcnn_fc_wstats_counts(out, int(bool(reset))))
+    return tuple(int(v) for v in out)
+
+
 def gemm_fixup_sites_reset():
     check(lib().kcnn_gemm_fixup_sites_reset())
 
diff --git a/kaldi-cnn_amd/src/capi/kcnn-capi.cc b/kaldi-cnn_amd/src/capi/kcnn-capi.cc
--- a/kaldi-cnn_amd/src/capi/kcnn-capi.cc
+++ b/kaldi-cnn_amd/src/capi/kcnn-capi.cc
@@ -107,21 +107,25 @@
   return u;
 }
 
-void param_ref(const kcnn_component *c, int which, float **data, MatrixDim *dim) {
+void param_ref(const kcnn_component *c, int which, float **data, MatrixDim *dim,
+               bool write = false) {
   using cnsl::nnet0::ConvolutionComponent;
   using cnsl::nnet0::FullyConnectedComponent;
   CuMatrixBase<BaseFloat> *m = nullptr;
   CuVectorBase<BaseFloat> *v = nullptr;
+  auto weights = [&](AffineComponent *a) {
+    return write ? &a->LinearParamsMutable() : const_cast<CuMatrix<BaseFloat> *>(&a->LinearParams());
+  };
   if (auto *cc = dynamic_cast<ConvolutionComponent *>(c->c)) {
     if (which == 0) m = &cc->LinearParamsMutable();
     else if (which == 1) v = &cc->BiasParamsMutable();
     else if (which == 2) m = &cc->PrevGradMutable();
   } else if (auto *fc = dynamic_cast<FullyConnectedComponent *>(c->c)) {
-    if (which == 0) m = &fc->LinearParamsMutable();
+    if (which == 0) m = weights(fc);
     else if (which == 1) v = &fc->BiasParamsMutable();
     else if (which == 2) m = &fc->PrevGradMutable();
   } else if (auto *af = dynamic_cast<AffineComponent *>(c->c)) {
-    if (which == 0) m = &af->LinearParamsMutable();
+    if (which == 0) m = weights(af);
     else if (which == 1) v = &af->BiasParamsMutable();
   }
   if (m) {
@@ -200,6 +204,11 @@
 int kcnn_gemm_fixup_counts(unsigned long long *out, int reset) {
   if (!out) return fail("kcnn_gemm_fixup_counts: out is NULL");
   kl_gemm_f16x3_fixup_counts(out, reset);
+  return 0;
+}
+int kcnn_fc_wstats_counts(unsigned long long *out, int reset) {
+  if (!out) return fail("kcnn_fc_wstats_counts: out is NULL");
+  kaldi::CuWeightStats::Counts(out, reset != 0);
   return 0;
 }
 int kcnn_gemm_fixup_sites_reset(void) {
@@ -526,7 +535,7 @@
   return guard([&] {
     float *p;
     MatrixDim d;
-    param_ref(c, which, &p, &d);
+    param_ref(c, which, &p, &d, true);
     copy2d(p, d, src, src_dim);
   });
 }
diff --git a/kaldi-cnn_amd/src/capi/nnet-stack.cc b/kaldi-cnn_amd/src/capi/nnet-stack.cc
--- a/kaldi-cnn_amd/src/capi/nnet-stack.cc
+++ b/kaldi-cnn_amd/src/capi/nnet-stack.cc
@@ -469,6 +469,7 @@
   CuSubMatrix<BaseFloat> od = out_deriv_of(i, out_deriv, od_dim);
   CuMatrix<BaseFloat> *dx = (i == 0 && skip_first_dx) ? nullptr : &c.deriv;
   ChunkInfo ii = in_info(i), oi = out_info(i);
+  auto wstats = c.affine->WeightStatsHint();
   CuGemmBackpropStats stats(od, c.affine->LinearParams(), true, &x);
   c.affine->BackpropGradient(ii, oi, x, y, od, nullptr, grad);
   if (between) between(ctx);
diff --git a/kaldi-cnn_amd/src/kaldi-lite/cu-f16-stats.hip b/kaldi-cnn_amd/src/kaldi-lite/cu-f16-stats.hip
--- a/kaldi-cnn_amd/src/kaldi-lite/cu-f16-stats.hip
+++ b/kaldi-cnn_amd/src/kaldi-lite/cu-f16-stats.hip
@@ -133,11 +133,13 @@
   }
 }
 
+template <bool RP>
 __device__ __forceinline__ void stats_cols(const StatOp &o, int blk) {
   const int cbi = blk % o.cb, rci = blk / o.cb;
   const int c0 = cbi * 1024 + threadIdx.x * 4;
   const int r0 = rci * o.rb, rend = min(o.rows, r0 + o.rb);
-  if (c0 >= o.cols) return;
+  const int lane = threadIdx.x & 63, piece = cbi * 4 + (threadIdx.x >> 6);
+  if (RP ? piece >= o.nwp : c0 >= o.cols) return;
   const bool v4 = o.vec && c0 + 4 <= o.cols;
   uint32_t cm[4] = {0u, 0u, 0u, 0u};
   uint32_t cn[4] = {0xffffffffu, 0xffffffffu, 0xffffffffu, 0xffffffffu};
@@ -145,17 +147,30 @@
     const float *x = X_row(o, r) + c0;
     if (v4) return *reinterpret_cast<const float4 *>(x);
     float4 q;
-    q.x = x[0];
+    q.x = c0 < o.cols ? x[0] : 0.0f;
     q.y = c0 + 1 < o.cols ? x[1] : 0.0f;
     q.z = c0 + 2 < o.cols ? x[2] : 0.0f;
     q.w = c0 + 3 < o.cols ? x[3] : 0.0f;
     return q;
   };
-  auto take = [&](float4 q) {
+  auto take = [&](int r, float4 q) {
     mm1(cm[0], cn[0], q.x);
     mm1(cm[1], cn[1], q.y);
     mm1(cm[2], cn[2], q.z);
     mm1(cm[3], cn[3], q.w);
+    if (RP) {
+      uint32_t m = 0, n = 0xffffffffu;
+      mm4(m, n, q);
+#pragma unroll
+      for (int d = 32; d >= 1; d >>= 1) {
+        m = max(m, (uint32_t)__shfl_xor((int)m, d));
+        n = min(n, (uint32_t)__shfl_xor((int)n, d));
+      }
+      if (lane == 0) {
+        o.rpart[(size_t)piece * o.rows + r] = m;
+        o.rpart[(size_t)(o.nwp + piece) * o.rows + r] = n;
+      }
+    }
   };
   int r = r0;
   for (; r + 8 <= rend; r += 8) {
@@ -163,9 +178,10 @@
 #pragma unroll
     for (int j = 0; j < 8; ++j) q[j] = load(r + j);
 #pragma unroll
-    for (int j = 0; j < 8; ++j) take(q[j]);
-  }
-  for (; r < rend; ++r) take(load(r));
+    for (int j = 0; j < 8; ++j) take(r + j, q[j]);
+  }
+  for (; r < rend; ++r) take(r, load(r));
+  if (c0 >= o.cols) return;
   uint32_t *dst = o.part + (size_t)rci * o.cols + c0;
   uint32_t *dsn = dst + (size_t)o.rbk * o.cols;
 #pragma unroll
@@ -189,9 +205,9 @@
   local = blk - n0 - n1;
   return 2;
 }
-__host__ __device__ inline int ncount_blocks(const StatOp &o);
+constexpr int FIN = 16;
 __host__ __device__ inline int nfinal_blocks(const StatOp &o) {
-  return o.mode == 1 && o.blocks ? o.fblocks : 0;
+  return o.mode == 1 && o.blocks ? o.fblocks + o.rfblocks : 0;
 }
 
 __global__ __launch_bounds__(256) void stats_kernel(StatOps s) {
@@ -207,11 +223,155 @@
   const int w = pick_op(s, blockIdx.x, [](const StatOp &o) { return o.blocks; }, blk);
   const StatOp &o = s.o[w];
   if (o.mode == 0) stats_rows(o, blk, red);
-  else stats_cols(o, blk);
+  else if (o.rpart) stats_cols<true>(o, blk);
+  else stats_cols<false>(o, blk);
+}
+
+struct FinSmem {
+  uint32_t red[2][FIN][FIN];
+  uint32_t susp[8];
+};
+__device__ __forceinline__ void fin_combine(FinSmem &sm, int g, int i, uint32_t &m, uint32_t &n) {
+  sm.red[0][g][i] = m;
+  sm.red[1][g][i] = n;
+  __syncthreads();
+  m = 0;
+  n = 0xffffffffu;
+#pragma unroll
+  for (int j = 0; j < FIN; ++j) {
+    m = max(m, sm.red[0][j][i]);
+    n = min(n, sm.red[1][j][i]);
+  }
+}
+__device__ __forceinline__ uint32_t fin_sum(FinSmem &sm, int g, int i, uint32_t cnt) {
+  sm.red[0][g][i] = cnt;
+  __syncthreads();
+  cnt = 0;
+#pragma unroll
+  for (int j = 0; j < FIN; ++j) cnt += sm.red[0][j][i];
+  return cnt;
+}
+__device__ __forceinline__ bool suspect(uint32_t b, float bound) {
+  return b != 0xffffffffu && __uint_as_float(b + 1u) < bound;
+}
+__device__ __forceinline__ uint32_t small1(float v, float bound) {
+  return (fabsf(v) < bound && v != 0.0f) ? 1u : 0u;
+}
+
+__device__ __forceinline__ void finish_cols(const StatOp &o, int blk, FinSmem &sm) {
+  const int i = threadIdx.x & (FIN - 1), g = threadIdx.x / FIN;
+  const int c = blk * FIN + i;
+  if (threadIdx.x < 8) sm.susp[threadIdx.x] = 0u;
+  const uint32_t *pm = o.part + c, *pn = o.part + (size_t)o.rbk * o.cols + c;
+  uint32_t m = 0, n = 0xffffffffu;
+  if (c < o.cols) {
+    int q = g;
+    for (; q + 7 * FIN < o.rbk; q += 8 * FIN) {
+      uint32_t a[8], b[8];
+#pragma unroll
+      for (int j = 0; j < 8; ++j) {
+        a[j] = pm[(size_t)(q + FIN * j) * o.cols];
+        b[j] = pn[(size_t)(q + FIN * j) * o.cols];
+      }
+#pragma unroll
+      for (int j = 0; j < 8; ++j) {
+        m = max(m, a[j]);
+        n = min(n, b[j]);
+      }
+    }
+    for (; q < o.rbk; q += FIN) {
+      m = max(m, pm[(size_t)q * o.cols]);
+      n = min(n, pn[(size_t)q * o.cols]);
+    }
+  }
+  fin_combine(sm, g, i, m, n);
+  const bool spr = c < o.cols && kcnn::f16x3::spread(m, n + 1u);
+  uint32_t cnt = 0;
+  if (__syncthreads_or(spr)) {
+    const float bound = spr ? kcnn::f16x3::small_bound(m) : 0.0f;
+    if (spr)
+      for (int q = g; q < o.rbk; q += 8 * FIN) {
+        uint32_t b[8];
+#pragma unroll
+        for (int j = 0; j < 8; ++j)
+          b[j] = q + FIN * j < o.rbk ? pn[(size_t)(q + FIN * j) * o.cols] : 0xffffffffu;
+#pragma unroll
+        for (int j = 0; j < 8; ++j)
+          if (suspect(b[j], bound)) atomicOr(&sm.susp[(q + FIN * j) >> 5], 1u << ((q + FIN * j) & 31));
+      }
+    __syncthreads();
+    for (int w = 0; w < 8; ++w)
+      for (uint32_t bits = sm.susp[w]; bits; bits &= bits - 1u) {
+        const int q = w * 32 + __builtin_ctz(bits);
+        const int r1 = min(o.rows, (q + 1) * o.rb);
+        for (int r = q * o.rb + g; r < r1; r += 16 * FIN) {
+          float v[16];
+#pragma unroll
+          for (int j = 0; j < 16; ++j)
+            v[j] = spr && r + FIN * j < r1 ? X_row(o, r + FIN * j)[c] : 0.0f;
+#pragma unroll
+          for (int j = 0; j < 16; ++j) cnt += small1(v[j], bound);
+        }
+      }
+    cnt = fin_sum(sm, g, i, cnt);
+  }
+  if (g == 0 && c < o.cols) {
+    o.out[c] = m;
+    o.out[o.cols + c] = n + 1u;
+    o.out[2 * (size_t)o.cols + c] = cnt;
+  }
+}
+
+__device__ __forceinline__ void finish_rows(const StatOp &o, int blk, FinSmem &sm) {
+  const int i = threadIdx.x & (FIN - 1), g = threadIdx.x / FIN, lane = threadIdx.x & 63;
+  const int r = blk * FIN + i;
+  const uint32_t *pm = o.rpart + r, *pn = o.rpart + (size_t)o.nwp * o.rows + r;
+  uint32_t m = 0, n = 0xffffffffu;
+  if (r < o.rows)
+    for (int p = g; p < o.nwp; p += FIN) {
+      m = max(m, pm[(size_t)p * o.rows]);
+      n = min(n, pn[(size_t)p * o.rows]);
+    }
+  fin_combine(sm, g, i, m, n);
+  const bool spr = r < o.rows && kcnn::f16x3::spread(m, n + 1u);
+  uint32_t cnt = 0;
+  if (__syncthreads_or(spr)) {
+    const float bound = spr ? kcnn::f16x3::small_bound(m) : 0.0f;
+    for (int p0 = 0; p0 < o.nwp; p0 += FIN) {
+      const int p = p0 + g;
+      const bool s = spr && p < o.nwp && suspect(pn[(size_t)p * o.rows], bound);
+      for (uint64_t mask = __ballot(s); mask; mask &= mask - 1u) {
+        const int src = __builtin_ctzll(mask);
+        const int pr = __shfl(r, src), pp = __shfl(p, src);
+        const float bd = __shfl(bound, src);
+        const int c0 = pp * 256 + lane * 4;
+        const float *x = X_row(o, pr) + c0;
+        float4 q = make_float4(0.0f, 0.0f, 0.0f, 0.0f);
+        if (o.vec && c0 + 4 <= o.cols) {
+          q = *reinterpret_cast<const float4 *>(x);
+        } else {
+          if (c0 < o.cols) q.x = x[0];
+          if (c0 + 1 < o.cols) q.y = x[1];
+          if (c0 + 2 < o.cols) q.z = x[2];
+          if (c0 + 3 < o.cols) q.w = x[3];
+        }
+        uint32_t k = small1(q.x, bd) + small1(q.y, bd) + small1(q.z, bd) + small1(q.w, bd);
+#pragma unroll
+        for (int d = 32; d >= 1; d >>= 1) k += (uint32_t)__shfl_xor((int)k, d);
+        if (lane == src) cnt += k;
+      }
+    }
+    cnt = fin_sum(sm, g, i, cnt);
+  }
+  if (g == 0 && r < o.rows) {
+    o.rout[r] = m;
+    o.rout[o.rows + r] = n + 1u;
+    o.rout[2 * (size_t)o.rows + r] = cnt;
+  }
 }
 
 __global__ __launch_bounds__(256) void stats_finalize_kernel(StatOps s) {
-  __shared__ uint32_t red[2][4][64];
+  __shared__ FinSmem sm;
   __shared__ PoolCountSmem psm;
   const int nf3 = nfinal_blocks(s.o[0]) + nfinal_blocks(s.o[1]) + nfinal_blocks(s.o[2]);
   if ((int)blockIdx.x >= nf3) {
@@ -221,74 +381,8 @@
   }
   int blk;
   const StatOp &o = s.o[pick_op(s, blockIdx.x, [](const StatOp &q) { return nfinal_blocks(q); }, blk)];
-  const int lane = threadIdx.x & 63, grp = threadIdx.x >> 6;
-  const int c = blk * 64 + lane;
-  uint32_t m = 0, n = 0xffffffffu;
-  if (c < o.cols) {
-    const uint32_t *pm = o.part + c, *pn = o.part + (size_t)o.rbk * o.cols + c;
-    int q = grp;
-    for (; q + 28 < o.rbk; q += 32) {
-      uint32_t a[8], b[8];
-#pragma unroll
-      for (int j = 0; j < 8; ++j) {
-        a[j] = pm[(size_t)(q + 4 * j) * o.cols];
-        b[j] = pn[(size_t)(q + 4 * j) * o.cols];
-      }
-#pragma unroll
-      for (int j = 0; j < 8; ++j) {
-        m = max(m, a[j]);
-        n = min(n, b[j]);
-      }
-    }
-    for (; q < o.rbk; q += 4) {
-      m = max(m, pm[(size_t)q * o.cols]);
-      n = min(n, pn[(size_t)q * o.cols]);
-    }
-  }
-  red[0][grp][lane] = m;
-  red[1][grp][lane] = n;
-  __syncthreads();
-  m = max(max(red[0][0][lane], red[0][1][lane]), max(red[0][2][lane], red[0][3][lane]));
-  n = min(min(red[1][0][lane], red[1][1][lane]), min(red[1][2][lane], red[1][3][lane]));
-  if (grp == 0 && c < o.cols) {
-    o.out[c] = m;
-    o.out[o.cols + c] = n + 1u;
-    o.out[2 * (size_t)o.cols + c] = 0;
-  }
-}
-
-constexpr int CNT_ROWS = 64;
-__host__ __device__ inline int ncount_blocks(const StatOp &o) {
-  return o.mode == 1 && o.blocks ? ((o.cols + 63) / 64) * ((o.rows + CNT_ROWS - 1) / CNT_ROWS) : 0;
-}
-__global__ __launch_bounds__(256) void stats_count_kernel(StatOps s) {
-  int blk;
-  const StatOp &o = s.o[pick_op(s, blockIdx.x, [](const StatOp &q) { return ncount_blocks(q); }, blk)];
-  const int ncb = (o.cols + 63) / 64;
-  const int cb = blk % ncb, rc = blk / ncb;
-  const int lane = threadIdx.x & 63, wave = threadIdx.x >> 6;
-  const int c = cb * 64 + lane;
-  bool spr = false;
-  float bound = 0.0f;
-  if (c < o.cols) {
-    const uint32_t mx = o.out[c];
-    spr = kcnn::f16x3::spread(mx, o.out[o.cols + c]);
-    if (spr) bound = kcnn::f16x3::small_bound(mx);
-  }
-  if (__ballot(spr) == 0) return;
-  const int r0 = rc * CNT_ROWS, r1 = min(o.rows, r0 + CNT_ROWS);
-  uint32_t cnt = 0;
-  if (spr) {
-    float v[CNT_ROWS / 4];
-#pragma unroll
-    for (int i = 0; i < CNT_ROWS / 4; ++i) {
-      const int r = r0 + wave + 4 * i;
-      v[i] = r < r1 ? fabsf(X_row(o, r)[c]) : 0.0f;
-    }
-#pragma unroll
-    for (int i = 0; i < CNT_ROWS / 4; ++i) cnt += (v[i] < bound && v[i] != 0.0f) ? 1u : 0u;
-  }
-  if (cnt) atomicAdd(o.out + 2 * (size_t)o.cols + c, cnt);
+  if (blk < o.fblocks) finish_cols(o, blk, sm);
+  else finish_rows(o, blk - o.fblocks, sm);
 }
 
 int stats_launch3(const StatOps &ops, hipStream_t st) {
@@ -297,22 +391,18 @@
       const size_t n = o.mode == 0 ? (size_t)std::max(o.rows, 0) : (size_t)std::max(o.cols, 0);
       if (n && hipMemsetAsync(o.out, 0, 3 * n * 4, st) != hipSuccess) return (int)hipGetLastError();
     }
-  int nb = 0, nf = 0, nc = 0;
+  int nb = 0, nf = 0;
   for (const StatOp &o : ops.o) {
     nb += o.blocks;
     nf += nfinal_blocks(o);
-    nc += ncount_blocks(o);
   }
   nb += ops.pcx * ops.pcy;
   nf += ops.pcn;
   if (nb == 0) return 0;
   hipLaunchKernelGGL(stats_kernel, dim3(nb), dim3(256), 0, st, ops);
-  int rc = kcnn::launch_status();
+  const int rc = kcnn::launch_status();
   if (rc || nf == 0) return rc;
   hipLaunchKernelGGL(stats_finalize_kernel, dim3(nf), dim3(256), 0, st, ops);
-  rc = kcnn::launch_status();
-  if (rc || nc == 0) return rc;
-  hipLaunchKernelGGL(stats_count_kernel, dim3(nc), dim3(256), 0, st, ops);
   return kcnn::launch_status();
 }
 
@@ -336,7 +426,7 @@
     o.rb = (rows + o.rbk - 1) / o.rbk;
     o.rbk = (rows + o.rb - 1) / o.rb;
     o.blocks = o.cb * o.rbk;
-    o.fblocks = (cols + 63) / 64;
+    o.fblocks = (cols + FIN - 1) / FIN;
   }
   return o;
 }
@@ -371,6 +461,30 @@
   if (rows > 0 && cols > 0 && !part) return (int)hipErrorInvalidValue;
   return stats_launch(stat_op(X, rows, cols, ld, 1, cmax, part), StatOp{},
                       kcnn::as_stream(stream));
+}
+
+extern "C" size_t kl_weight_stats_words(int rows, int cols) {
+  if (rows <= 0 || cols <= 0) return 0;
+  return stat_part_words(rows, cols, 1) + 2 * (size_t)((cols + 255) / 256) * rows;
+}
+extern "C" int kl_weight_stats(const float *W, int rows, int cols, int ld, uint32_t *rmax,
+                               uint32_t *cmax, uint32_t *part, kcnn_stream_t stream) {
+  if (rows < 0 || cols < 0 || ld < cols || !rmax || !cmax) return (int)hipErrorInvalidValue;
+  hipStream_t st = kcnn::as_stream(stream);
+  if (rows == 0 || cols == 0) {
+    if (rows && hipMemsetAsync(rmax, 0, 3 * (size_t)rows * 4, st) != hipSuccess)
+      return (int)hipGetLastError();
+    if (cols && hipMemsetAsync(cmax, 0, 3 * (size_t)cols * 4, st) != hipSuccess)
+      return (int)hipGetLastError();
+    return 0;
+  }
+  if (!part) return (int)hipErrorInvalidValue;
+  StatOp o = stat_op(W, rows, cols, ld, 1, cmax, part);
+  o.rout = rmax;
+  o.rpart = part + stat_part_words(rows, cols, 1);
+  o.nwp = (cols + 255) / 256;
+  o.rfblocks = (rows + FIN - 1) / FIN;
+  return stats_launch(o, StatOp{}, st);
 }
 
 extern "C" int kl_absmax_rows_cols(const float *R, int rows, int cols, int ld, uint32_t *rmax,
diff --git a/kaldi-cnn_amd/src/kaldi-lite/cu-kernels-lite.h b/kaldi-cnn_amd/src/kaldi-lite/cu-kernels-lite.h
--- a/kaldi-cnn_amd/src/kaldi-lite/cu-kernels-lite.h
+++ b/kaldi-cnn_amd/src/kaldi-lite/cu-kernels-lite.h
@@ -30,6 +30,9 @@
 size_t kl_absmax_cols_words(int rows, int cols);
 int kl_absmax_cols(const float *X, int rows, int cols, int ld, uint32_t *cmax, uint32_t *part,
                    kcnn_stream_t st);
+size_t kl_weight_stats_words(int rows, int cols);
+int kl_weight_stats(const float *W, int rows, int cols, int ld, uint32_t *rmax, uint32_t *cmax,
+                    uint32_t *part, kcnn_stream_t stream);
 int kl_absmax_rows_cols(const float *R, int rows, int cols, int ld, uint32_t *rmax,
                         const float *Q, int qrows, int qcols, int ldq, uint32_t *cmax,
                         uint32_t *part, uint32_t *clear, kcnn_stream_t stream);
diff --git a/kaldi-cnn_amd/src/kaldi-lite/cu-matrix.cc b/kaldi-cnn_amd/src/kaldi-lite/cu-matrix.cc
--- a/kaldi-cnn_amd/src/kaldi-lite/cu-matrix.cc
+++ b/kaldi-cnn_amd/src/kaldi-lite/cu-matrix.cc
@@ -5,6 +5,7 @@
 #include <stdlib.h>
 #include <string.h>
 
+#include <atomic>
 #include <limits>
 #include <mutex>
 #include <sstream>
@@ -285,12 +286,14 @@
   CuDevice &dev = CuDevice::Instantiate();
   const int N = dy.NumRows(), O = dy.NumCols(), I = W.NumCols();
   if (dev.GemmMode() < 2 || N == 0 || O == 0 || I == 0 || W.NumRows() != O) return;
+  const CuGemmStatsHint *hw = CuGemmStatsHint::Find(W.Data(), O, I, W.Stride());
+  const bool w_known = hw && hw->colmax && !hw->pending;
   {
     const CuGemmStatsHint *hd = CuGemmStatsHint::Find(dy.Data(), N, O, dy.Stride());
-    const CuGemmStatsHint *hw = CuGemmStatsHint::Find(W.Data(), O, I, W.Stride());
-    if (hd && hd->rowmax && (!cols || hd->colmax) && hw && hw->colmax && !hw->pending) return;
-  }
-  const size_t pd = cols ? kl_absmax_cols_words(N, O) : 0, pw = kl_absmax_cols_words(O, I);
+    if (hd && hd->rowmax && (!cols || hd->colmax) && w_known) return;
+  }
+  const size_t pd = cols ? kl_absmax_cols_words(N, O) : 0,
+               pw = w_known ? 0 : kl_absmax_cols_words(O, I);
   const size_t words = 3 * ((size_t)N + O + I) + pd + pw;
   ws_ = dev.Malloc(words * 4);
   uint32_t *rows_d = static_cast<uint32_t *>(ws_), *cols_d = rows_d + 3 * (size_t)N,
@@ -304,11 +307,49 @@
   }
   CNSL_SAFE_CALL(kl_gemm_stats3(dy.Data(), N, O, dy.Stride(), 0, rows_d, nullptr,
                                 cols ? dy.Data() : nullptr, N, O, dy.Stride(), 1, cols_d, part_d,
-                                W.Data(), O, I, W.Stride(), 1, cols_w, part_w, pc,
-                                reinterpret_cast<kcnn_stream_t>(dev.Stream())));
+                                w_known ? nullptr : W.Data(), O, I, W.Stride(), 1, cols_w, part_w,
+                                pc, reinterpret_cast<kcnn_stream_t>(dev.Stream())));
   if (pc) pc->pending = 0;
   hint_d_ = new CuGemmStatsHint(dy.Data(), N, O, dy.Stride(), rows_d, cols ? cols_d : nullptr);
-  hint_w_ = new CuGemmStatsHint(W.Data(), O, I, W.Stride(), nullptr, cols_w);
+  if (!w_known) hint_w_ = new CuGemmStatsHint(W.Data(), O, I, W.Stride(), nullptr, cols_w);
+}
+
+static std::atomic<unsigned long long> g_wstats_computed{0}, g_wstats_reused{0};
+
+CuWeightStats::~CuWeightStats() {
+  if (buf_) CuDevice::Instantiate().Free(buf_);
+}
+void CuWeightStats::Counts(unsigned long long *out, bool reset) {
+  out[0] = reset ? g_wstats_computed.exchange(0) : g_wstats_computed.load();
+  out[1] = reset ? g_wstats_reused.exchange(0) : g_wstats_reused.load();
+}
+std::unique_ptr<CuGemmStatsHint> CuWeightStats::Hint(const CuMatrixBase<float> &W) {
+  CuDevice &dev = CuDevice::Instantiate();
+  const MatrixIndexT O = W.NumRows(), I = W.NumCols();
+  if (dev.GemmMode() < 2 || O == 0 || I == 0) return nullptr;
+  std::lock_guard<std::mutex> lk(mu_);
+  if (valid_ && (O != rows_ || I != cols_)) valid_ = false;
+  if (!valid_) {
+    if (!buf_ || O != rows_ || I != cols_) {
+      if (buf_) dev.Free(buf_);
+      buf_ = dev.Malloc(3 * ((size_t)O + I) * 4);
+      rows_ = O;
+      cols_ = I;
+    }
+    const size_t pw = kl_weight_stats_words(O, I);
+    uint32_t *part = static_cast<uint32_t *>(dev.Malloc(pw * 4));
+    uint32_t *rows = static_cast<uint32_t *>(buf_);
+    CNSL_SAFE_CALL(kl_weight_stats(W.Data(), O, I, W.Stride(), rows, rows + 3 * (size_t)O, part,
+                                   reinterpret_cast<kcnn_stream_t>(dev.Stream())));
+    dev.Free(part);
+    valid_ = true;
+    g_wstats_computed++;
+  } else {
+    g_wstats_reused++;
+  }
+  uint32_t *rows = static_cast<uint32_t *>(buf_);
+  return std::unique_ptr<CuGemmStatsHint>(
+      new CuGemmStatsHint(W.Data(), O, I, W.Stride(), rows, rows + 3 * (size_t)O));
 }
 CuGemmBackpropStats::~CuGemmBackpropStats() {
   delete hint_w_;
diff --git a/kaldi-cnn_amd/src/kaldi-lite/cu-matrix.h b/kaldi-cnn_amd/src/kaldi-lite/cu-matrix.h
--- a/kaldi-cnn_amd/src/kaldi-lite/cu-matrix.h
+++ b/kaldi-cnn_amd/src/kaldi-lite/cu-matrix.h
@@ -2,6 +2,8 @@
 #define KCNN_KALDI_LITE_CU_MATRIX_H_
 
 #include <istream>
+#include <memory>
+#include <mutex>
 #include <ostream>
 #include <vector>
 
@@ -284,6 +286,23 @@
   const CuGemmStatsHint *prev_;
 };
 
+class CuWeightStats {
+ public:
+  CuWeightStats() {}
+  CuWeightStats(const CuWeightStats &) {}
+  CuWeightStats &operator=(const CuWeightStats &) { Invalidate(); return *this; }
+  ~CuWeightStats();
+  void Invalidate() { valid_ = false; }
+  std::unique_ptr<CuGemmStatsHint> Hint(const CuMatrixBase<float> &W);
+  static void Counts(unsigned long long *out, bool reset);
+
+ private:
+  std::mutex mu_;
+  void *buf_ = nullptr;
+  MatrixIndexT rows_ = 0, cols_ = 0;
+  bool valid_ = false;
+};
+
 class CuGemmBackpropStats {
  public:
   CuGemmBackpropStats(const CuMatrixBase<float> &out_deriv, const CuMatrixBase<float> &linear,
diff --git a/kaldi-cnn_amd/src/kaldi-lite/f16-stats.h b/kaldi-cnn_amd/src/kaldi-lite/f16-stats.h
--- a/kaldi-cnn_amd/src/kaldi-lite/f16-stats.h
+++ b/kaldi-cnn_amd/src/kaldi-lite/f16-stats.h
@@ -11,11 +11,13 @@
   const float *X;
   uint32_t *out;
   uint32_t *part;
+  uint32_t *rout, *rpart;
   int rows, cols, ld, mode, vec;
   int blocks;
   int rpb;
   int cb, rbk, rb;
   int fblocks;
+  int nwp, rfblocks;
   uint32_t *clear;
 };
 
diff --git a/kaldi-cnn_amd/src/nnet0/nnet-component-nnet0.cc b/kaldi-cnn_amd/src/nnet0/nnet-component-nnet0.cc
--- a/kaldi-cnn_amd/src/nnet0/nnet-component-nnet0.cc
+++ b/kaldi-cnn_amd/src/nnet0/nnet-component-nnet0.cc
@@ -1015,7 +1015,7 @@
   ExpectOneOrTwoTokens(is, binary, ostr_beg.str(), "<LearningRate>");
   ReadBasicType(is, binary, &learning_rate_);
   ExpectToken(is, binary, "<LinearParams>");
-  linear_params_.Read(is, binary);
+  MutableW().Read(is, binary);
   ExpectToken(is, binary, "<BiasParams>");
   bias_params_.Read(is, binary);
   ExpectToken(is, binary, "<WeightDecay>");
@@ -1035,7 +1035,7 @@
   WriteToken(os, binary, "<LearningRate>");
   WriteBasicType(os, binary, learning_rate_);
   WriteToken(os, binary, "<LinearParams>");
-  linear_params_.Write(os, binary);
+  W().Write(os, binary);
   WriteToken(os, binary, "<BiasParams>");
   bias_params_.Write(os, binary);
   WriteToken(os, binary, "<WeightDecay>");
@@ -1053,11 +1053,11 @@
                                    BaseFloat weight_decay, BaseFloat momentum) {
   UpdatableComponent::Init(learning_rate);
   KALDI_ASSERT(input_dim > 0 && output_dim > 0);
-  linear_params_.Resize(output_dim, input_dim);
+  MutableW().Resize(output_dim, input_dim);
   bias_params_.Resize(output_dim);
   KALDI_ASSERT(output_dim > 0 && input_dim > 0 && param_stddev >= 0.0);
-  linear_params_.SetRandn();
-  linear_params_.Scale(param_stddev);
+  MutableW().SetRandn();
+  MutableW().Scale(param_stddev);
   bias_params_.SetZero();
   bias_params_.Add(bias_stddev);
   weight_decay_ = weight_decay;
@@ -1095,8 +1095,8 @@
 
 std::string FullyConnectedComponent::Info() const {
   std::stringstream stream;
-  const double size = (double)linear_params_.NumRows() * linear_params_.NumCols();
-  const double ls = std::sqrt(TraceMatMat(linear_params_, linear_params_, kTrans) / size);
+  const double size = (double)W().NumRows() * W().NumCols();
+  const double ls = std::sqrt(TraceMatMat(W(), W(), kTrans) / size);
   const double bs = std::sqrt(VecVec(bias_params_, bias_params_) / bias_params_.Dim());
   stream << Type() << ", input-dim=" << InputDim()
          << ", output-dim=" << OutputDim() << ", linear-params-stddev=" << ls
@@ -1109,7 +1109,7 @@
 Component *FullyConnectedComponent::Copy() const {
   FullyConnectedComponent *ans = new FullyConnectedComponent();
   ans->learning_rate_ = learning_rate_;
-  ans->linear_params_ = linear_params_;
+  ans->MutableW() = W();
   ans->bias_params_ = bias_params_;
   ans->weight_decay_ = weight_decay_;
   ans->momentum_ = momentum_;
@@ -1138,7 +1138,7 @@
   const BaseFloat a_wd = (BaseFloat)(-1 * learning_rate * weight_decay_);
   const BaseFloat a_g = (BaseFloat)learning_rate;
   CNSL_SAFE_CALL(hipF_momentum_update(
-      linear_params_.Data(), linear_params_.Dim(), prev_grad_.Data(),
+      MutableW().Data(), W().Dim(), prev_grad_.Data(),
       prev_grad_.Dim(), grad, Dense(OutputDim(), InputDim()), momentum_, a_wd,
       a_g, bias_params_.Data(), grad + (size_t)OutputDim() * InputDim(),
       OutputDim(), S()));
@@ -1151,9 +1151,9 @@
     const double learning_rate = learning_rate_ / (double)num_sample;
     bias_params_.AddRowSumMat(learning_rate, out_deriv, 1.0);
     prev_grad_.Scale(momentum_);
-    prev_grad_.AddMat(-1 * learning_rate * weight_decay_, linear_params_, kNoTrans);
+    prev_grad_.AddMat(-1 * learning_rate * weight_decay_, W(), kNoTrans);
     prev_grad_.AddMatMat(learning_rate, out_deriv, kTrans, in_value, kNoTrans, 1.0);
-    linear_params_.AddMat(1.0, prev_grad_, kNoTrans);
+    MutableW().AddMat(1.0, prev_grad_, kNoTrans);
     return;
   }
   {
@@ -1161,7 +1161,7 @@
     const BaseFloat a_wd = (BaseFloat)(-1 * learning_rate * weight_decay_);
     const BaseFloat a_g = (BaseFloat)learning_rate;
     CuProfileScope prof("FullyConnectedComponent::ComputeGradient");
-    if (linear_params_.AddMatMatMomentum(out_deriv, kTrans, in_value, kNoTrans, &prev_grad_,
+    if (MutableW().AddMatMatMomentum(out_deriv, kTrans, in_value, kNoTrans, &prev_grad_,
                                          momentum_, a_wd, a_g)) {
       bias_params_.AddRowSumMat(a_g, out_deriv, 1.0);
       return;
diff --git a/kaldi-cnn_amd/src/nnet2/nnet-component.cc b/kaldi-cnn_amd/src/nnet2/nnet-component.cc
--- a/kaldi-cnn_amd/src/nnet2/nnet-component.cc
+++ b/kaldi-cnn_amd/src/nnet2/nnet-component.cc
@@ -191,17 +191,17 @@
 
 AffineComponent::AffineComponent(const AffineComponent &component)
     : UpdatableComponent(component),
-      linear_params_(component.linear_params_),
       bias_params_(component.bias_params_),
-      is_gradient_(component.is_gradient_) {}
+      is_gradient_(component.is_gradient_),
+      linear_params_(component.linear_params_) {}
 
 AffineComponent::AffineComponent(const CuMatrixBase<BaseFloat> &linear_params,
                                  const CuVectorBase<BaseFloat> &bias_params,
                                  BaseFloat learning_rate)
     : UpdatableComponent(learning_rate),
-      linear_params_(linear_params),
       bias_params_(),
-      is_gradient_(false) {
+      is_gradient_(false),
+      linear_params_(linear_params) {
   bias_params_ = bias_params;
   KALDI_ASSERT(linear_params.NumRows() == bias_params.Dim() &&
                bias_params.Dim() != 0);
@@ -211,11 +211,11 @@
                            int32 output_dim, BaseFloat param_stddev,
                            BaseFloat bias_stddev) {
   UpdatableComponent::Init(learning_rate);
-  linear_params_.Resize(output_dim, input_dim);
+  MutableW().Resize(output_dim, input_dim);
   bias_params_.Resize(output_dim);
   KALDI_ASSERT(output_dim > 0 && input_dim > 0 && param_stddev >= 0.0);
-  linear_params_.SetRandn();
-  linear_params_.Scale(param_stddev);
+  MutableW().SetRandn();
+  MutableW().Scale(param_stddev);
   bias_params_.SetRandn();
   bias_params_.Scale(bias_stddev);
 }
@@ -240,8 +240,8 @@
 
 std::string AffineComponent::Info() const {
   std::stringstream stream;
-  const double size = (double)linear_params_.NumRows() * linear_params_.NumCols();
-  const double ls = std::sqrt(TraceMatMat(linear_params_, linear_params_, kTrans) / size);
+  const double size = (double)W().NumRows() * W().NumCols();
+  const double ls = std::sqrt(TraceMatMat(W(), W(), kTrans) / size);
   const double bs = std::sqrt(VecVec(bias_params_, bias_params_) / bias_params_.Dim());
   stream << Type() << ", input-dim=" << InputDim()
          << ", output-dim=" << OutputDim() << ", linear-params-stddev=" << ls
@@ -257,26 +257,26 @@
   in_info.CheckSize(in);
   out_info.CheckSize(*out);
   KALDI_ASSERT(in_info.NumChunks() == out_info.NumChunks());
-  out->AddMatMatBias(1.0, in, kNoTrans, linear_params_, kTrans, bias_params_);
+  auto wstats = WeightStatsHint();
+  out->AddMatMatBias(1.0, in, kNoTrans, W(), kTrans, bias_params_);
 }
 
 void AffineComponent::Scale(BaseFloat scale) {
-  linear_params_.Scale(scale);
+  MutableW().Scale(scale);
   bias_params_.Scale(scale);
 }
 
 void AffineComponent::Add(BaseFloat alpha, const UpdatableComponent &other_in) {
   const AffineComponent *other = dynamic_cast<const AffineComponent *>(&other_in);
   KALDI_ASSERT(other != NULL);
-  linear_params_.AddMat(alpha, other->linear_params_);
+  MutableW().AddMat(alpha, other->W());
   bias_params_.AddVec(alpha, other->bias_params_);
 }
 
 void AffineComponent::UpdateSimple(const CuMatrixBase<BaseFloat> &in_value,
                                    const CuMatrixBase<BaseFloat> &out_deriv) {
   bias_params_.AddRowSumMat(learning_rate_, out_deriv, 1.0);
-  linear_params_.AddMatMat(learning_rate_, out_deriv, kTrans, in_value,
-                           kNoTrans, 1.0);
+  MutableW().AddMatMat(learning_rate_, out_deriv, kTrans, in_value, kNoTrans, 1.0);
 }
 
 void AffineComponent::Backprop(const ChunkInfo &, const ChunkInfo &,
@@ -287,8 +287,9 @@
                                CuMatrix<BaseFloat> *in_deriv) const {
   AffineComponent *to_update = dynamic_cast<AffineComponent *>(to_update_in);
   in_deriv->Resize(out_deriv.NumRows(), InputDim(), kUndefined);
-  CuGemmBackpropStats stats(out_deriv, linear_params_, to_update != NULL, &in_value);
-  in_deriv->AddMatMat(1.0, out_deriv, kNoTrans, linear_params_, kNoTrans, 0.0);
+  auto wstats = WeightStatsHint();
+  CuGemmBackpropStats stats(out_deriv, W(), to_update != NULL, &in_value);
+  in_deriv->AddMatMat(1.0, out_deriv, kNoTrans, W(), kNoTrans, 0.0);
   if (to_update != NULL) {
     if (to_update->is_gradient_)
       to_update->UpdateSimple(in_value, out_deriv);
@@ -302,7 +303,7 @@
     SetLearningRate(1.0);
     is_gradient_ = true;
   }
-  linear_params_.SetZero();
+  MutableW().SetZero();
   bias_params_.SetZero();
 }
 
@@ -313,7 +314,7 @@
   ExpectOneOrTwoTokens(is, binary, ostr_beg.str(), "<LearningRate>");
   ReadBasicType(is, binary, &learning_rate_);
   ExpectToken(is, binary, "<LinearParams>");
-  linear_params_.Read(is, binary);
+  MutableW().Read(is, binary);
   ExpectToken(is, binary, "<BiasParams>");
   bias_params_.Read(is, binary);
   std::string tok;
@@ -343,7 +344,7 @@
   WriteToken(os, binary, "<LearningRate>");
   WriteBasicType(os, binary, learning_rate_);
   WriteToken(os, binary, "<LinearParams>");
-  linear_params_.Write(os, binary);
+  W().Write(os, binary);
   WriteToken(os, binary, "<BiasParams>");
   bias_params_.Write(os, binary);
   WriteToken(os, binary, "<IsGradient>");
@@ -354,23 +355,23 @@
 BaseFloat AffineComponent::DotProduct(const UpdatableComponent &other_in) const {
   const AffineComponent *other = dynamic_cast<const AffineComponent *>(&other_in);
   KALDI_ASSERT(other != NULL);
-  return TraceMatMat(linear_params_, other->linear_params_, kTrans) +
+  return TraceMatMat(W(), other->W(), kTrans) +
          VecVec(bias_params_, other->bias_params_);
 }
 
 Component *AffineComponent::Copy() const {
   AffineComponent *ans = new AffineComponent();
   ans->learning_rate_ = learning_rate_;
-  ans->linear_params_ = linear_params_;
+  ans->MutableW() = W();
   ans->bias_params_ = bias_params_;
   ans->is_gradient_ = is_gradient_;
   return ans;
 }
 
 void AffineComponent::PerturbParams(BaseFloat stddev) {
-  CuMatrix<BaseFloat> temp_linear_params(linear_params_);
+  CuMatrix<BaseFloat> temp_linear_params(W());
   temp_linear_params.SetRandn();
-  linear_params_.AddMat(stddev, temp_linear_params);
+  MutableW().AddMat(stddev, temp_linear_params);
   CuVector<BaseFloat> temp_bias_params(bias_params_);
   temp_bias_params.SetRandn();
   bias_params_.AddVec(stddev, temp_bias_params);
@@ -379,8 +380,8 @@
 void AffineComponent::SetParams(const VectorBase<BaseFloat> &bias,
                                 const MatrixBase<BaseFloat> &linear) {
   bias_params_ = bias;
-  linear_params_ = linear;
-  KALDI_ASSERT(bias_params_.Dim() == linear_params_.NumRows());
+  MutableW() = linear;
+  KALDI_ASSERT(bias_params_.Dim() == W().NumRows());
 }
 
 int32 AffineComponent::GetParameterDim() const {
@@ -388,22 +389,22 @@
 }
 void AffineComponent::Vectorize(VectorBase<BaseFloat> *params) const {
   KALDI_ASSERT(params->Dim() == GetParameterDim());
-  Matrix<BaseFloat> W;
-  linear_params_.CopyToMat(&W);
+  Matrix<BaseFloat> Wh;
+  W().CopyToMat(&Wh);
   Vector<BaseFloat> b;
   bias_params_.CopyToVec(&b);
   const size_t nw = (size_t)InputDim() * OutputDim();
-  std::copy(W.Data(), W.Data() + nw, params->Data());
+  std::copy(Wh.Data(), Wh.Data() + nw, params->Data());
   std::copy(b.Data(), b.Data() + OutputDim(), params->Data() + nw);
 }
 void AffineComponent::UnVectorize(const VectorBase<BaseFloat> &params) {
   KALDI_ASSERT(params.Dim() == GetParameterDim());
-  Matrix<BaseFloat> W(OutputDim(), InputDim());
+  Matrix<BaseFloat> Wh(OutputDim(), InputDim());
   const size_t nw = (size_t)InputDim() * OutputDim();
-  std::copy(params.Data(), params.Data() + nw, W.Data());
+  std::copy(params.Data(), params.Data() + nw, Wh.Data());
   Vector<BaseFloat> b(OutputDim());
   std::copy(params.Data() + nw, params.Data() + nw + OutputDim(), b.Data());
-  linear_params_.CopyFromMat(W);
+  MutableW().CopyFromMat(Wh);
   bias_params_.CopyFromVec(b);
 }
 
diff --git a/kaldi-cnn_amd/src/nnet2/nnet-component.h b/kaldi-cnn_amd/src/nnet2/nnet-component.h
--- a/kaldi-cnn_amd/src/nnet2/nnet-component.h
+++ b/kaldi-cnn_amd/src/nnet2/nnet-component.h
@@ -147,8 +147,8 @@
                   const CuVectorBase<BaseFloat> &bias_params,
                   BaseFloat learning_rate);
   AffineComponent() : is_gradient_(false) {}
-  virtual int32 InputDim() const { return linear_params_.NumCols(); }
-  virtual int32 OutputDim() const { return linear_params_.NumRows(); }
+  virtual int32 InputDim() const { return W().NumCols(); }
+  virtual int32 OutputDim() const { return W().NumRows(); }
   void Init(BaseFloat learning_rate, int32 input_dim, int32 output_dim,
             BaseFloat param_stddev, BaseFloat bias_stddev);
   virtual void InitFromString(std::string args);
@@ -177,15 +177,22 @@
   virtual void SetParams(const VectorBase<BaseFloat> &bias,
                          const MatrixBase<BaseFloat> &linear);
   const CuVector<BaseFloat> &BiasParams() { return bias_params_; }
-  const CuMatrix<BaseFloat> &LinearParams() { return linear_params_; }
+  const CuMatrix<BaseFloat> &LinearParams() const { return W(); }
   virtual int32 GetParameterDim() const;
   virtual void Vectorize(VectorBase<BaseFloat> *params) const;
   virtual void UnVectorize(const VectorBase<BaseFloat> &params);
 
-  CuMatrix<BaseFloat> &LinearParamsMutable() { return linear_params_; }
+  CuMatrix<BaseFloat> &LinearParamsMutable() { return MutableW(); }
   CuVector<BaseFloat> &BiasParamsMutable() { return bias_params_; }
 
+  std::unique_ptr<CuGemmStatsHint> WeightStatsHint() const { return wstats_.Hint(W()); }
+
  protected:
+  const CuMatrix<BaseFloat> &W() const { return linear_params_; }
+  CuMatrix<BaseFloat> &MutableW() {
+    wstats_.Invalidate();
+    return linear_params_;
+  }
   virtual void Update(const CuMatrixBase<BaseFloat> &in_value,
                       const CuMatrixBase<BaseFloat> &out_deriv) {
     UpdateSimple(in_value, out_deriv);
@@ -194,9 +201,12 @@
                             const CuMatrixBase<BaseFloat> &out_deriv);
   const AffineComponent &operator=(const AffineComponent &other);
 
-  CuMatrix<BaseFloat> linear_params_;
   CuVector<BaseFloat> bias_params_;
   bool is_gradient_;
+
+ private:
+  CuMatrix<BaseFloat> linear_params_;
+  mutable CuWeightStats wstats_;
 };
 
 
```

Result: no change. 3.131 million frames/sec, median of 6 (+0.8%).
